# HySonLab/EquiHGNN

Measured on AMD Instinct MI355X. Metric: training molecules/sec on QM9 egnn_equihnns, higher is better.
Workload: dtype f32; 1 GPU; qm9-like synthetic molecules, --method egnn_equihnns, batch 256/rank, hidden 256, 3 layers (scripts/run_qm9_3d.sh); full training step fwd+MSE+bwd+all-reduce+Adam; batch_per_rank=256, global_batch=256, parallelism=dp1, launch=hipGraph replay (padded static shapes), collective=none (single rank)

## Files before the change

equihgnn_amd/csrc/egnn_edge.hip:

```cpp
#include <cstdlib>

#include "act.h"
#include "common.h"
#include "bf16x3.h"
#include "mfma.h"

namespace {

constexpr int KNB = 16;
constexpr int MDIM = 16;
constexpr int THREADS = 256;
constexpr int WAVES = THREADS / 64;

__device__ __forceinline__ f32x2 silu_fast2(f32x2 x) {
    const f32x2 t = x * f32x2{-1.442695041f, -1.442695041f};
    const f32x2 d = f32x2{__builtin_amdgcn_exp2f(t.x), __builtin_amdgcn_exp2f(t.y)} + f32x2{1.0f, 1.0f};
    return x * f32x2{__builtin_amdgcn_rcpf(d.x), __builtin_amdgcn_rcpf(d.y)};
}
__device__ __forceinline__ float silu_grad(float x, float* ds) {
    const float sig = sigmoid_fast(x);
    const float s = x * sig;
    *ds = fmaf(s, 1.0f - sig, sig);
    return s;
}

__device__ __forceinline__ int xcd_item(int b, int grid, int n_items, int remap) {
    if (!remap) return b < n_items ? b : -1;
    const int per = grid >> 3;
    const int item = (b & 7) * per + (b >> 3);
    return item < n_items ? item : -1;
}
static inline int xcd_grid(int n_items, int remap) { return remap ? ((n_items + 7) / 8) * 8 : n_items; }

__host__ __device__ inline int lds_row_stride(int Hp) {
    return Hp + ((24 - (Hp & 63)) + 64) % 64;
}

constexpr int FWD_THREADS = 1024;
constexpr int FWD_SPLIT = 4;
constexpr int FWD_NODES = FWD_THREADS / 64 / FWD_SPLIT;
constexpr int FWD_UB = 4;
constexpr int FWD_LD = 16 * FWD_UB + 4;
constexpr int FWD_TILE = (KNB + 1) * FWD_LD;

template <int NU>
__device__ __forceinline__ f32x4 fwd_stage(const float* __restrict__ t_rd, const float* __restrict__ t_rda,
                                           const float* __restrict__ wrow, const float* __restrict__ crow,
                                           float dd, f32x4 acc) {
    const f32x2 dd2 = {dd, dd};
#pragma unroll
    for (int u = 0; u < NU; ++u) {
        const float4 b4 = *reinterpret_cast<const float4*>(t_rd + 16 * u);
        const float4 a4 = *reinterpret_cast<const float4*>(t_rda + 16 * u);
        const float4 w4 = *reinterpret_cast<const float4*>(wrow + 16 * u);
        const float4 c4 = *reinterpret_cast<const float4*>(crow + 16 * u);
        const f32x2 h01 = f32x2{c4.x, c4.y} * dd2 + (f32x2{a4.x, a4.y} + f32x2{b4.x, b4.y});
        const f32x2 h23 = f32x2{c4.z, c4.w} * dd2 + (f32x2{a4.z, a4.w} + f32x2{b4.z, b4.w});
        const f32x2 s01 = silu_fast2(h01);
        const f32x2 s23 = silu_fast2(h23);
        acc = mfma16(s01.x, w4.x, acc);
        acc = mfma16(s01.y, w4.y, acc);
        acc = mfma16(s23.x, w4.z, acc);
        acc = mfma16(s23.y, w4.w, acc);
    }
    return acc;
}

template <bool W2_LDS>
__global__ void __launch_bounds__(FWD_THREADS)
k_edge_fwd(const float* __restrict__ ab, const float* __restrict__ wd, const float* __restrict__ w2,
           const float* __restrict__ b2, const int* __restrict__ nbr, const float* __restrict__ d2,
           float* __restrict__ m, float* __restrict__ pre2, int N, int Hp) {
    extern __shared__ __attribute__((aligned(16))) float s_mem[];
    const int ldw = W2_LDS ? lds_row_stride(Hp) : Hp;
    float* s_w2 = s_mem;
    float* s_wd = s_w2 + (W2_LDS ? MDIM * ldw : 0);
    float* s_tile = s_wd + Hp;
    if (W2_LDS) {
        for (int idx = threadIdx.x * 4; idx < MDIM * Hp; idx += FWD_THREADS * 4) {
            const int o = idx / Hp, k = idx - o * Hp;
            *reinterpret_cast<float4*>(s_w2 + o * ldw + k) = *reinterpret_cast<const float4*>(w2 + idx);
        }
    }
    for (int idx = threadIdx.x * 4; idx < Hp; idx += FWD_THREADS * 4)
        *reinterpret_cast<float4*>(s_wd + idx) = *reinterpret_cast<const float4*>(wd + idx);
    __syncthreads();
    const int lane = threadIdx.x & 63;
    const int wave = __builtin_amdgcn_readfirstlane(threadIdx.x >> 6);
    const int r = lane & 15, q = lane >> 4;
    const int slot = wave / FWD_SPLIT, part = wave % FWD_SPLIT;
    const int per = (Hp >> 4) / FWD_SPLIT;
    const int s_beg = part * per;
    const int nfull = per / FWD_UB, tail = per % FWD_UB;
    const int nstages = nfull + (tail ? 1 : 0);
    const float bo = b2[r];
    const float* __restrict__ wrow = (W2_LDS ? s_w2 : w2) + r * ldw + 4 * q + 16 * s_beg;
    const float* __restrict__ crow = s_wd + 4 * q + 16 * s_beg;
    float* tile = s_tile + wave * FWD_TILE;
    float* t_wr = tile + q * FWD_LD + 4 * r;
    const float* t_rd = tile + r * FWD_LD + 4 * q;
    const float* t_rda = tile + KNB * FWD_LD + 4 * q;
    float* t_wra = tile + KNB * FWD_LD + 4 * r;
    const int groups = (N + FWD_NODES - 1) / FWD_NODES;
    const int gpb = (groups + gridDim.x - 1) / gridDim.x;
    const int g_beg = blockIdx.x * gpb;
    const int g_end = (g_beg + gpb < groups) ? g_beg + gpb : groups;
    const int b_col0 = 16 * s_beg + 4 * r;
    if (g_beg >= g_end) return;
    const int bc0 = (b_col0 < Hp - 4) ? b_col0 : Hp - 4;
    int node_raw = g_beg * FWD_NODES + slot;
    int node = (node_raw < N) ? node_raw : N - 1;
    float dd = d2[node * KNB + r];
    const float* __restrict__ arow = ab + (int64_t)node * 2 * Hp;
    const float* __restrict__ brow0 = ab + (int64_t)nbr[node * KNB + q] * 2 * Hp + Hp;
    const float* __restrict__ brow1 = ab + (int64_t)nbr[node * KNB + 4 + q] * 2 * Hp + Hp;
    const float* __restrict__ brow2 = ab + (int64_t)nbr[node * KNB + 8 + q] * 2 * Hp + Hp;
    const float* __restrict__ brow3 = ab + (int64_t)nbr[node * KNB + 12 + q] * 2 * Hp + Hp;
    float4 nb0 = *reinterpret_cast<const float4*>(brow0 + bc0);
    float4 nb1 = *reinterpret_cast<const float4*>(brow1 + bc0);
    float4 nb2 = *reinterpret_cast<const float4*>(brow2 + bc0);
    float4 nb3 = *reinterpret_cast<const float4*>(brow3 + bc0);
    float4 na = make_float4(0.f, 0.f, 0.f, 0.f);
    if (q == 0) na = *reinterpret_cast<const float4*>(arow + bc0);
    for (int group = g_beg; group < g_end; ++group) {
        f32x4 acc = {0.f, 0.f, 0.f, 0.f};
        int j0 = 0, j1 = 0, j2 = 0, j3 = 0, node_raw_n = 0, node_n = 0;
        float dd_n = 0.f;
        for (int st = 0; st < nstages; ++st) {
            *reinterpret_cast<float4*>(t_wr) = nb0;
            *reinterpret_cast<float4*>(t_wr + 4 * FWD_LD) = nb1;
            *reinterpret_cast<float4*>(t_wr + 8 * FWD_LD) = nb2;
            *reinterpret_cast<float4*>(t_wr + 12 * FWD_LD) = nb3;
            if (q == 0) *reinterpret_cast<float4*>(t_wra) = na;
            if (st == 0) {
                const int gn = (group + 1 < g_end) ? group + 1 : group;
                node_raw_n = gn * FWD_NODES + slot;
                node_n = (node_raw_n < N) ? node_raw_n : N - 1;
                j0 = nbr[node_n * KNB + q];
                j1 = nbr[node_n * KNB + 4 + q];
                j2 = nbr[node_n * KNB + 8 + q];
                j3 = nbr[node_n * KNB + 12 + q];
                dd_n = d2[node_n * KNB + r];
            }
            const float* __restrict__ p0 = brow0;
            const float* __restrict__ p1 = brow1;
            const float* __restrict__ p2 = brow2;
            const float* __restrict__ p3 = brow3;
            const float* __restrict__ pa = arow;
            int bc;
            if (st + 1 < nstages) {
                const int off = 16 * FWD_UB * (st + 1);
                bc = (b_col0 + off < Hp - 4) ? b_col0 + off : Hp - 4;
            } else {
                asm volatile("" : "+v"(j0), "+v"(j1), "+v"(j2), "+v"(j3), "+v"(node_n));
                p0 = ab + (int64_t)j0 * 2 * Hp + Hp;
                p1 = ab + (int64_t)j1 * 2 * Hp + Hp;
                p2 = ab + (int64_t)j2 * 2 * Hp + Hp;
                p3 = ab + (int64_t)j3 * 2 * Hp + Hp;
                pa = ab + (int64_t)node_n * 2 * Hp;
                bc = bc0;
            }
            nb0 = *reinterpret_cast<const float4*>(p0 + bc);
            nb1 = *reinterpret_cast<const float4*>(p1 + bc);
            nb2 = *reinterpret_cast<const float4*>(p2 + bc);
            nb3 = *reinterpret_cast<const float4*>(p3 + bc);
            if (q == 0) na = *reinterpret_cast<const float4*>(pa + bc);
            __builtin_amdgcn_sched_barrier(0);
            const float* wr = wrow + 16 * FWD_UB * st;
            const float* cr = crow + 16 * FWD_UB * st;
            if (st < nfull) acc = fwd_stage<FWD_UB>(t_rd, t_rda, wr, cr, dd, acc);
            else if (tail == 1) acc = fwd_stage<1>(t_rd, t_rda, wr, cr, dd, acc);
            else if (tail == 2) acc = fwd_stage<2>(t_rd, t_rda, wr, cr, dd, acc);
            else acc = fwd_stage<3>(t_rd, t_rda, wr, cr, dd, acc);
            __builtin_amdgcn_sched_barrier(0);
            if (st + 1 == nstages) { brow0 = p0; brow1 = p1; brow2 = p2; brow3 = p3; arow = pa; }
        }
        if (part > 0) *reinterpret_cast<f32x4*>(tile + lane * 4) = acc;
        __syncthreads();
        if (part == 0 && node_raw < N) {
#pragma unroll
            for (int pp = 1; pp < FWD_SPLIT; ++pp)
                acc += *reinterpret_cast<const f32x4*>(tile + pp * FWD_TILE + lane * 4);
            float msum = 0.f;
#pragma unroll
            for (int g = 0; g < 4; ++g) {
                const float pv = acc[g] + bo;
                pre2[(int64_t)node * (KNB * MDIM) + (4 * q + g) * MDIM + r] = pv;
                msum += silu_fast(pv);
            }
            msum += __shfl_xor(msum, 16, 64);
            msum += __shfl_xor(msum, 32, 64);
            if (q == 0) m[(int64_t)node * MDIM + r] = msum;
        }
        __syncthreads();
        node_raw = node_raw_n;
        node = node_n;
        dd = dd_n;
    }
}

constexpr int edge_planes(int np) { return np == 6 ? 3 : (np == 3 ? 2 : 1); }

constexpr int F2_SPLIT = 4;
constexpr int F2_LD = 32 + 4;
constexpr int F2_TILE = (KNB + 1) * F2_LD;
constexpr int F2_MAXSTEPS = 9;

template <int PL>
__device__ __forceinline__ void split8(const float (&v)[8], uint4& p0, uint4& p1, uint4& p2) {
    split_pair_n<PL>(v[0], v[1], p0.x, p1.x, p2.x);
    split_pair_n<PL>(v[2], v[3], p0.y, p1.y, p2.y);
    split_pair_n<PL>(v[4], v[5], p0.z, p1.z, p2.z);
    split_pair_n<PL>(v[6], v[7], p0.w, p1.w, p2.w);
}

template <int NS, int THREADS_, bool W2_LDS, int NP>
__global__ void __launch_bounds__(THREADS_)
k_edge_fwd_x3(const float* __restrict__ ab, const float* __restrict__ wd, const float* __restrict__ w2,
              const float* __restrict__ b2, const int* __restrict__ nbr, const float* __restrict__ d2,
              float* __restrict__ m, float* __restrict__ pre2, int N, int Hp, int n_items, int remap) {
    extern __shared__ __attribute__((aligned(16))) float s_mem[];
    constexpr int NWAVES = THREADS_ / 64, NODES = NWAVES / F2_SPLIT, PL = edge_planes(NP);
    const int item = xcd_item((int)blockIdx.x, (int)gridDim.x, n_items, remap);
    if (item < 0) return;
    const int total = Hp >> 5;
    float* s_wd = s_mem;
    float* s_tile = s_wd + Hp;
    uint4* s_w2 = reinterpret_cast<uint4*>(s_tile + NWAVES * F2_TILE);
    for (int idx = threadIdx.x * 4; idx < Hp; idx += THREADS_ * 4)
        *reinterpret_cast<float4*>(s_wd + idx) = *reinterpret_cast<const float4*>(wd + idx);
    const int lane = threadIdx.x & 63;
    const int wave = __builtin_amdgcn_readfirstlane(threadIdx.x >> 6);
    const int r = lane & 15, q = lane >> 4;
    const int slot = wave / F2_SPLIT, part = wave % F2_SPLIT;
    const int per = (total + F2_SPLIT - 1) / F2_SPLIT;
    const int s_beg = part * per;
    const int cnt = (total - s_beg < per) ? (total - s_beg > 0 ? total - s_beg : 0) : per;
    auto w2_frag = [&](int step, uint4& p0, uint4& p1, uint4& p2) {
        float v[8];
        const int k0 = 32 * step + 8 * q;
        const float4 x0 = *reinterpret_cast<const float4*>(w2 + r * Hp + k0);
        const float4 x1 = *reinterpret_cast<const float4*>(w2 + r * Hp + k0 + 4);
        v[0] = x0.x; v[1] = x0.y; v[2] = x0.z; v[3] = x0.w; v[4] = x1.x; v[5] = x1.y; v[6] = x1.z; v[7] = x1.w;
        split8<PL>(v, p0, p1, p2);
    };
    uint4 wf[W2_LDS ? 1 : NS][3];
    if constexpr (W2_LDS) {
        for (int step = wave; step < total; step += NWAVES) {
            uint4 p0, p1, p2;
            w2_frag(step, p0, p1, p2);
            s_w2[(step * 3 + 0) * 64 + lane] = p0;
            if constexpr (PL > 1) s_w2[(step * 3 + 1) * 64 + lane] = p1;
            if constexpr (PL > 2) s_w2[(step * 3 + 2) * 64 + lane] = p2;
        }
    } else {
#pragma unroll
        for (int s = 0; s < NS; ++s) {
            if (s < cnt) w2_frag(s_beg + s, wf[s][0], wf[s][1], wf[s][2]);
            else wf[s][0] = wf[s][1] = wf[s][2] = make_uint4(0u, 0u, 0u, 0u);
        }
    }
    __syncthreads();
    const float bo = b2[r];
    float* tile = s_tile + wave * F2_TILE;
    const int lrow = lane >> 3, piece = lane & 7;
    float* t_wr0 = tile + lrow * F2_LD + 4 * piece;
    float* t_wr1 = t_wr0 + 8 * F2_LD;
    float* t_wra = tile + KNB * F2_LD + 4 * piece;
    const float* t_rd = tile + r * F2_LD + 8 * q;
    const float* t_rda = tile + KNB * F2_LD + 8 * q;
    const int groups = (N + NODES - 1) / NODES;
    const int gpb = (groups + n_items - 1) / n_items;
    const int g_beg = item * gpb;
    const int g_end = (g_beg + gpb < groups) ? g_beg + gpb : groups;
    if (g_beg >= g_end) return;
    const int col0 = 32 * s_beg + 4 * piece;
    int node_raw = g_beg * NODES + slot;
    int node = (node_raw < N) ? node_raw : N - 1;
    float dd = d2[node * KNB + r];
    const float* __restrict__ arow = ab + (int64_t)node * 2 * Hp;
    const float* __restrict__ brow0 = ab + (int64_t)nbr[node * KNB + lrow] * 2 * Hp + Hp;
    const float* __restrict__ brow1 = ab + (int64_t)nbr[node * KNB + 8 + lrow] * 2 * Hp + Hp;
    float4 nb0 = f4_zero(), nb1 = f4_zero(), na = f4_zero();
    if (cnt > 0) {
        nb0 = *reinterpret_cast<const float4*>(brow0 + col0);
        nb1 = *reinterpret_cast<const float4*>(brow1 + col0);
        if (lane < 8) na = *reinterpret_cast<const float4*>(arow + col0);
    }
    for (int group = g_beg; group < g_end; ++group) {
        f32x4 acc = {0.f, 0.f, 0.f, 0.f};
        int j0 = 0, j1 = 0, node_raw_n = 0, node_n = 0;
        float dd_n = 0.f;
        {
            const int gn = (group + 1 < g_end) ? group + 1 : group;
            node_raw_n = gn * NODES + slot;
            node_n = (node_raw_n < N) ? node_raw_n : N - 1;
            j0 = nbr[node_n * KNB + lrow];
            j1 = nbr[node_n * KNB + 8 + lrow];
            dd_n = d2[node_n * KNB + r];
        }
#pragma unroll
        for (int st = 0; st < NS; ++st) {
            if (st < cnt) {
                *reinterpret_cast<float4*>(t_wr0) = nb0;
                *reinterpret_cast<float4*>(t_wr1) = nb1;
                if (lane < 8) *reinterpret_cast<float4*>(t_wra) = na;
                const float* __restrict__ p0 = brow0;
                const float* __restrict__ p1 = brow1;
                const float* __restrict__ pa = arow;
                int bc;
                if (st + 1 < cnt) {
                    bc = col0 + 32 * (st + 1);
                } else {
                    asm volatile("" : "+v"(j0), "+v"(j1), "+v"(node_n));
                    p0 = ab + (int64_t)j0 * 2 * Hp + Hp;
                    p1 = ab + (int64_t)j1 * 2 * Hp + Hp;
                    pa = ab + (int64_t)node_n * 2 * Hp;
                    bc = col0;
                }
                nb0 = *reinterpret_cast<const float4*>(p0 + bc);
                nb1 = *reinterpret_cast<const float4*>(p1 + bc);
                if (lane < 8) na = *reinterpret_cast<const float4*>(pa + bc);
                if (st + 1 >= cnt) { brow0 = p0; brow1 = p1; arow = pa; }
                __builtin_amdgcn_sched_barrier(0);
                const float* cr = s_wd + 32 * (s_beg + st) + 8 * q;
                const float4 b0 = *reinterpret_cast<const float4*>(t_rd), b1 = *reinterpret_cast<const float4*>(t_rd + 4);
                const float4 a0 = *reinterpret_cast<const float4*>(t_rda), a1 = *reinterpret_cast<const float4*>(t_rda + 4);
                const float4 c0 = *reinterpret_cast<const float4*>(cr), c1 = *reinterpret_cast<const float4*>(cr + 4);
#ifdef EDGE_ABLATE
                acc[0] += (b0.x + b1.w) + (a0.y + a1.z) + (c0.x + c1.x);
                __builtin_amdgcn_sched_barrier(0);
                continue;
#endif
                const f32x2 dd2 = {dd, dd};
                const f32x2 s01 = silu_fast2(f32x2{c0.x, c0.y} * dd2 + (f32x2{a0.x, a0.y} + f32x2{b0.x, b0.y}));
                const f32x2 s23 = silu_fast2(f32x2{c0.z, c0.w} * dd2 + (f32x2{a0.z, a0.w} + f32x2{b0.z, b0.w}));
                const f32x2 s45 = silu_fast2(f32x2{c1.x, c1.y} * dd2 + (f32x2{a1.x, a1.y} + f32x2{b1.x, b1.y}));
                const f32x2 s67 = silu_fast2(f32x2{c1.z, c1.w} * dd2 + (f32x2{a1.z, a1.w} + f32x2{b1.z, b1.w}));
                uint4 p0_, p1_, p2_;
                split_pair_n<PL>(s01.x, s01.y, p0_.x, p1_.x, p2_.x);
                split_pair_n<PL>(s23.x, s23.y, p0_.y, p1_.y, p2_.y);
                split_pair_n<PL>(s45.x, s45.y, p0_.z, p1_.z, p2_.z);
                split_pair_n<PL>(s67.x, s67.y, p0_.w, p1_.w, p2_.w);
                const bf16x8 x0 = __builtin_bit_cast(bf16x8, p0_), x1 = __builtin_bit_cast(bf16x8, p1_), x2 = __builtin_bit_cast(bf16x8, p2_);
                uint4 q0, q1 = make_uint4(0u, 0u, 0u, 0u), q2 = q1;
                if constexpr (W2_LDS) {
                    const uint4* wp = s_w2 + (s_beg + st) * 3 * 64 + lane;
                    q0 = wp[0];
                    if constexpr (PL > 1) q1 = wp[64];
                    if constexpr (PL > 2) q2 = wp[128];
                } else {
                    q0 = wf[st][0]; q1 = wf[st][1]; q2 = wf[st][2];
                }
                const bf16x8 w0 = __builtin_bit_cast(bf16x8, q0), w1 = __builtin_bit_cast(bf16x8, q1), w2p = __builtin_bit_cast(bf16x8, q2);
                if constexpr (NP == 6) {
                    acc = __builtin_amdgcn_mfma_f32_16x16x32_bf16(x1, w1, acc, 0, 0, 0);
                    acc = __builtin_amdgcn_mfma_f32_16x16x32_bf16(x0, w2p, acc, 0, 0, 0);
                    acc = __builtin_amdgcn_mfma_f32_16x16x32_bf16(x2, w0, acc, 0, 0, 0);
                    acc = __builtin_amdgcn_mfma_f32_16x16x32_bf16(x0, w1, acc, 0, 0, 0);
                    acc = __builtin_amdgcn_mfma_f32_16x16x32_bf16(x1, w0, acc, 0, 0, 0);
                } else if constexpr (NP == 3) {
                    acc = __builtin_amdgcn_mfma_f32_16x16x32_bf16(x1, w0, acc, 0, 0, 0);
                    acc = __builtin_amdgcn_mfma_f32_16x16x32_bf16(x0, w1, acc, 0, 0, 0);
                }
                acc = __builtin_amdgcn_mfma_f32_16x16x32_bf16(x0, w0, acc, 0, 0, 0);
                __builtin_amdgcn_sched_barrier(0);
            }
        }
        if (part > 0) *reinterpret_cast<f32x4*>(tile + lane * 4) = acc;
        __syncthreads();
        if (part == 0 && node_raw < N) {
#pragma unroll
            for (int pp = 1; pp < F2_SPLIT; ++pp)
                acc += *reinterpret_cast<const f32x4*>(tile + pp * F2_TILE + lane * 4);
            float msum = 0.f;
#pragma unroll
            for (int g = 0; g < 4; ++g) {
                const float pv = acc[g] + bo;
                pre2[(int64_t)node * (KNB * MDIM) + (4 * q + g) * MDIM + r] = pv;
                msum += silu_fast(pv);
            }
            msum += __shfl_xor(msum, 16, 64);
            msum += __shfl_xor(msum, 32, 64);
            if (q == 0) m[(int64_t)node * MDIM + r] = msum;
        }
        __syncthreads();
        node_raw = node_raw_n;
        node = node_n;
        dd = dd_n;
    }
}

template <int NP>
__device__ __forceinline__ f32x4 mfma16_planes(const Planes4& a, const Planes4& b, f32x4 c) {
    if constexpr (NP == 3) {
        c = mfma16_bf16(a.p1, b.p0, c);
        c = mfma16_bf16(a.p0, b.p1, c);
    }
    return mfma16_bf16(a.p0, b.p0, c);
}
template <int NP>
__device__ __forceinline__ void w2_planes(const float4& w0, const float4& w1, const float4& w2v, const float4& w3, Planes4& c0,
                                          Planes4& c1, Planes4& c2, Planes4& c3) {
    constexpr int PL = edge_planes(NP);
    c0 = split_quad<PL>(w0.x, w1.x, w2v.x, w3.x);
    c1 = split_quad<PL>(w0.y, w1.y, w2v.y, w3.y);
    c2 = split_quad<PL>(w0.z, w1.z, w2v.z, w3.z);
    c3 = split_quad<PL>(w0.w, w1.w, w2v.w, w3.w);
}
constexpr int BW_RESIDENT = 768;

__host__ __device__ inline int bw_chunks(int64_t n_items, int tiles) {
    int64_t c = BW_RESIDENT / tiles;
    if (c < 1) c = 1;
    const int64_t most = (n_items + WAVES - 1) / WAVES;
    if (c > most) c = most;
    return (int)(c < 1 ? 1 : c);
}

__global__ void __launch_bounds__(THREADS)
k_edge_bwd_prep(const float* __restrict__ pre2, const float* __restrict__ dm, float* __restrict__ dpre2,
                float* __restrict__ dpre2_t, const int* __restrict__ t_perm, const int* __restrict__ nbr,
                const float* __restrict__ d2, int4* __restrict__ rec, float* __restrict__ slab_b2, int N, int64_t dm_ld) {
    const int64_t E = (int64_t)N * KNB;
    for (int64_t p = (int64_t)blockIdx.x * THREADS + threadIdx.x; p < E; p += (int64_t)gridDim.x * THREADS) {
        const int e = t_perm[p];
        rec[p] = make_int4(e, nbr[e], __float_as_int(d2[e]), 0);
    }
    const int lane = threadIdx.x & 63, wave = threadIdx.x >> 6;
    float4 acc_b2 = f4_zero();
    for (int node = blockIdx.x * WAVES + wave; node < N; node += gridDim.x * WAVES) {
        const int jj = lane >> 2, o0 = (lane & 3) * 4;
        const float4 p4 = *reinterpret_cast<const float4*>(pre2 + (int64_t)node * 256 + lane * 4);
        const float4 g4 = *reinterpret_cast<const float4*>(dm + (int64_t)node * dm_ld + o0);
        float ds;
        float4 d4;
        silu_grad(p4.x, &ds); d4.x = g4.x * ds;
        silu_grad(p4.y, &ds); d4.y = g4.y * ds;
        silu_grad(p4.z, &ds); d4.z = g4.z * ds;
        silu_grad(p4.w, &ds); d4.w = g4.w * ds;
        *reinterpret_cast<float4*>(dpre2 + (int64_t)node * 256 + lane * 4) = d4;
        float* __restrict__ t = dpre2_t + (int64_t)node * 256 + jj;
        t[(o0 + 0) * KNB] = d4.x;
        t[(o0 + 1) * KNB] = d4.y;
        t[(o0 + 2) * KNB] = d4.z;
        t[(o0 + 3) * KNB] = d4.w;
        f4_add(acc_b2, d4);
    }
    if (slab_b2) {
#pragma unroll
        for (int off = 4; off < 64; off <<= 1) {
            acc_b2.x += __shfl_xor(acc_b2.x, off); acc_b2.y += __shfl_xor(acc_b2.y, off);
            acc_b2.z += __shfl_xor(acc_b2.z, off); acc_b2.w += __shfl_xor(acc_b2.w, off);
        }
        __shared__ float4 s_b2[WAVES][4];
        if (lane < 4) s_b2[wave][lane] = acc_b2;
        __syncthreads();
        if (threadIdx.x < 4) {
            float4 v = s_b2[0][threadIdx.x];
            for (int w = 1; w < WAVES; ++w) f4_add(v, s_b2[w][threadIdx.x]);
            *reinterpret_cast<float4*>(slab_b2 + (int64_t)blockIdx.x * MDIM + 4 * threadIdx.x) = v;
        }
    }
}

struct RecvOps {
    float4 pa;
    float4 pt;
    float4 a;
    float4 dd;
    float4 b0, b1, b2, b3;
};

__device__ __forceinline__ void recv_load(RecvOps& o, const float* __restrict__ ab, const float* __restrict__ d2,
                                          const float* __restrict__ dpre2, const float* __restrict__ dpre2_t,
                                          int node, int4 nb, int Hp, int k4, int r, int q) {
    o.pa = *reinterpret_cast<const float4*>(dpre2 + (int64_t)node * 256 + r * MDIM + 4 * q);
    o.pt = *reinterpret_cast<const float4*>(dpre2_t + (int64_t)node * 256 + r * KNB + 4 * q);
    o.a = *reinterpret_cast<const float4*>(ab + (int64_t)node * 2 * Hp + k4);
    o.dd = *reinterpret_cast<const float4*>(d2 + (int64_t)node * KNB + 4 * q);
    o.b0 = *reinterpret_cast<const float4*>(ab + (int64_t)nb.x * 2 * Hp + Hp + k4);
    o.b1 = *reinterpret_cast<const float4*>(ab + (int64_t)nb.y * 2 * Hp + Hp + k4);
    o.b2 = *reinterpret_cast<const float4*>(ab + (int64_t)nb.z * 2 * Hp + Hp + k4);
    o.b3 = *reinterpret_cast<const float4*>(ab + (int64_t)nb.w * 2 * Hp + Hp + k4);
}

template <int NP>
__device__ __forceinline__ float recv_column(float a, float wdc, const float4& dd, float b0, float b1, float b2,
                                             float b3, const f32x4& gk, const float4& pt, const Planes4& ptp, float& acc_wd,
                                             f32x4& acc_w) {
    float ds0, ds1, ds2, ds3;
    const float s0 = silu_grad(fmaf(wdc, dd.x, a + b0), &ds0);
    const float s1 = silu_grad(fmaf(wdc, dd.y, a + b1), &ds1);
    const float s2 = silu_grad(fmaf(wdc, dd.z, a + b2), &ds2);
    const float s3 = silu_grad(fmaf(wdc, dd.w, a + b3), &ds3);
    const float dh0 = gk[0] * ds0, dh1 = gk[1] * ds1, dh2 = gk[2] * ds2, dh3 = gk[3] * ds3;
    acc_wd = fmaf(dh0, dd.x, acc_wd);
    acc_wd = fmaf(dh1, dd.y, acc_wd);
    acc_wd = fmaf(dh2, dd.z, acc_wd);
    acc_wd = fmaf(dh3, dd.w, acc_wd);
    if constexpr (NP == 6) {
        acc_w = mfma16(pt.x, s0, acc_w);
        acc_w = mfma16(pt.y, s1, acc_w);
        acc_w = mfma16(pt.z, s2, acc_w);
        acc_w = mfma16(pt.w, s3, acc_w);
    } else {
        acc_w = mfma16_planes<NP>(ptp, split_quad<edge_planes(NP)>(s0, s1, s2, s3), acc_w);
    }
    return (dh0 + dh1) + (dh2 + dh3);
}

template <int NP>
__global__ void __launch_bounds__(THREADS)
k_edge_bwd_recv(const float* __restrict__ ab, const float* __restrict__ wd, const float* __restrict__ w2,
                const int* __restrict__ nbr, const float* __restrict__ d2, const float* __restrict__ dpre2,
                const float* __restrict__ dpre2_t, float* __restrict__ dab, float* __restrict__ slab_w2,
                float* __restrict__ slab_wd, int N, int Hp, int tiles, int chunk_nodes, int n_items, int remap) {
    __shared__ __attribute__((aligned(16))) float s_red[WAVES - 1][64 * 20];
    const int lane = threadIdx.x & 63;
    const int wave = __builtin_amdgcn_readfirstlane(threadIdx.x >> 6);
    const int r = lane & 15, q = lane >> 4;
    const int item = xcd_item((int)blockIdx.x, (int)gridDim.x, n_items, remap);
    if (item < 0) return;
    const int T = item % tiles, chunk = item / tiles;
    const int base = chunk * chunk_nodes;
    const int cnt = (N - base < chunk_nodes) ? (N - base) : chunk_nodes;
    const int k4 = 64 * T + 4 * r;
    const float4 w0 = *reinterpret_cast<const float4*>(w2 + (4 * q + 0) * Hp + k4);
    const float4 w1 = *reinterpret_cast<const float4*>(w2 + (4 * q + 1) * Hp + k4);
    const float4 w2v = *reinterpret_cast<const float4*>(w2 + (4 * q + 2) * Hp + k4);
    const float4 w3 = *reinterpret_cast<const float4*>(w2 + (4 * q + 3) * Hp + k4);
    const float4 wd4 = *reinterpret_cast<const float4*>(wd + k4);
    Planes4 wp0 = {}, wp1 = {}, wp2 = {}, wp3 = {};
    if constexpr (NP != 6) w2_planes<NP>(w0, w1, w2v, w3, wp0, wp1, wp2, wp3);
    f32x4 aw0 = {0.f, 0.f, 0.f, 0.f}, aw1 = aw0, aw2 = aw0, aw3 = aw0;
    float ad0 = 0.f, ad1 = 0.f, ad2 = 0.f, ad3 = 0.f;
    const int last = cnt - 1;
    int n = wave;
    if (n < cnt) {
        const int4* __restrict__ nbr4 = reinterpret_cast<const int4*>(nbr);
        auto clampn = [&](int x) { return base + (x < last ? x : last); };
        int4 nb_next = nbr4[(int64_t)clampn(n) * 4 + q];
        RecvOps nx;
        recv_load(nx, ab, d2, dpre2, dpre2_t, clampn(n), nb_next, Hp, k4, r, q);
        nb_next = nbr4[(int64_t)clampn(n + WAVES) * 4 + q];
        for (; n < cnt; n += WAVES) {
            const RecvOps cur = nx;
            const int node = base + n;
            recv_load(nx, ab, d2, dpre2, dpre2_t, clampn(n + WAVES), nb_next, Hp, k4, r, q);
            nb_next = nbr4[(int64_t)clampn(n + 2 * WAVES) * 4 + q];
            __builtin_amdgcn_sched_barrier(0);
#ifdef EDGE_ABLATE
            {
                const float t = (cur.pa.x + cur.pt.y) + (cur.a.x + cur.dd.y) + ((cur.b0.x + cur.b1.y) + (cur.b2.z + cur.b3.w));
                if (q == 0) *reinterpret_cast<float4*>(dab + (int64_t)node * 2 * Hp + k4) = make_float4(t, t, t, t);
                ad0 += t;
                continue;
            }
#endif
            f32x4 g0 = {0.f, 0.f, 0.f, 0.f}, g1 = g0, g2 = g0, g3 = g0;
            Planes4 ptp = {};
            if constexpr (NP == 6) {
                g0 = mfma16(cur.pa.x, w0.x, g0); g1 = mfma16(cur.pa.x, w0.y, g1);
                g2 = mfma16(cur.pa.x, w0.z, g2); g3 = mfma16(cur.pa.x, w0.w, g3);
                g0 = mfma16(cur.pa.y, w1.x, g0); g1 = mfma16(cur.pa.y, w1.y, g1);
                g2 = mfma16(cur.pa.y, w1.z, g2); g3 = mfma16(cur.pa.y, w1.w, g3);
                g0 = mfma16(cur.pa.z, w2v.x, g0); g1 = mfma16(cur.pa.z, w2v.y, g1);
                g2 = mfma16(cur.pa.z, w2v.z, g2); g3 = mfma16(cur.pa.z, w2v.w, g3);
                g0 = mfma16(cur.pa.w, w3.x, g0); g1 = mfma16(cur.pa.w, w3.y, g1);
                g2 = mfma16(cur.pa.w, w3.z, g2); g3 = mfma16(cur.pa.w, w3.w, g3);
            } else {
                const Planes4 pap = split_quad<edge_planes(NP)>(cur.pa.x, cur.pa.y, cur.pa.z, cur.pa.w);
                g0 = mfma16_planes<NP>(pap, wp0, g0); g1 = mfma16_planes<NP>(pap, wp1, g1);
                g2 = mfma16_planes<NP>(pap, wp2, g2); g3 = mfma16_planes<NP>(pap, wp3, g3);
                ptp = split_quad<edge_planes(NP)>(cur.pt.x, cur.pt.y, cur.pt.z, cur.pt.w);
            }
            float da0 = recv_column<NP>(cur.a.x, wd4.x, cur.dd, cur.b0.x, cur.b1.x, cur.b2.x, cur.b3.x, g0, cur.pt, ptp, ad0, aw0);
            float da1 = recv_column<NP>(cur.a.y, wd4.y, cur.dd, cur.b0.y, cur.b1.y, cur.b2.y, cur.b3.y, g1, cur.pt, ptp, ad1, aw1);
            float da2 = recv_column<NP>(cur.a.z, wd4.z, cur.dd, cur.b0.z, cur.b1.z, cur.b2.z, cur.b3.z, g2, cur.pt, ptp, ad2, aw2);
            float da3 = recv_column<NP>(cur.a.w, wd4.w, cur.dd, cur.b0.w, cur.b1.w, cur.b2.w, cur.b3.w, g3, cur.pt, ptp, ad3, aw3);
            da0 += __shfl_xor(da0, 16, 64); da1 += __shfl_xor(da1, 16, 64);
            da2 += __shfl_xor(da2, 16, 64); da3 += __shfl_xor(da3, 16, 64);
            da0 += __shfl_xor(da0, 32, 64); da1 += __shfl_xor(da1, 32, 64);
            da2 += __shfl_xor(da2, 32, 64); da3 += __shfl_xor(da3, 32, 64);
            if (q == 0)
                *reinterpret_cast<float4*>(dab + (int64_t)node * 2 * Hp + k4) = make_float4(da0, da1, da2, da3);
            __builtin_amdgcn_sched_barrier(0);
        }
    }
    ad0 += __shfl_xor(ad0, 16, 64); ad1 += __shfl_xor(ad1, 16, 64);
    ad2 += __shfl_xor(ad2, 16, 64); ad3 += __shfl_xor(ad3, 16, 64);
    ad0 += __shfl_xor(ad0, 32, 64); ad1 += __shfl_xor(ad1, 32, 64);
    ad2 += __shfl_xor(ad2, 32, 64); ad3 += __shfl_xor(ad3, 32, 64);
    if (wave > 0) {
        float* p = &s_red[wave - 1][lane * 20];
        *reinterpret_cast<f32x4*>(p) = aw0;
        *reinterpret_cast<f32x4*>(p + 4) = aw1;
        *reinterpret_cast<f32x4*>(p + 8) = aw2;
        *reinterpret_cast<f32x4*>(p + 12) = aw3;
        *reinterpret_cast<float4*>(p + 16) = make_float4(ad0, ad1, ad2, ad3);
    }
    __syncthreads();
    if (wave == 0) {
#pragma unroll
        for (int w = 0; w < WAVES - 1; ++w) {
            const float* p = &s_red[w][lane * 20];
            aw0 += *reinterpret_cast<const f32x4*>(p);
            aw1 += *reinterpret_cast<const f32x4*>(p + 4);
            aw2 += *reinterpret_cast<const f32x4*>(p + 8);
            aw3 += *reinterpret_cast<const f32x4*>(p + 12);
            const float4 d = *reinterpret_cast<const float4*>(p + 16);
            ad0 += d.x; ad1 += d.y; ad2 += d.z; ad3 += d.w;
        }
        float* __restrict__ sw = slab_w2 + (int64_t)chunk * (MDIM + 1) * Hp;
#pragma unroll
        for (int g = 0; g < 4; ++g)
            *reinterpret_cast<float4*>(sw + (4 * q + g) * Hp + k4) = make_float4(aw0[g], aw1[g], aw2[g], aw3[g]);
        if (q == 0)
            *reinterpret_cast<float4*>(slab_wd + (int64_t)chunk * (MDIM + 1) * Hp + k4) = make_float4(ad0, ad1, ad2, ad3);
    }
}

constexpr int SEND_LD = 68;

struct SendOps {
    float4 pa;
    float4 a0, a1, a2, a3;
    float4 b0, b1, b2, b3;
    float dd0, dd1, dd2, dd3;
};

__device__ __forceinline__ void send_load(SendOps& o, const float* __restrict__ ab,
                                          const float* __restrict__ dpre2, int4 rc, int Hp, int k4, int q) {
    o.pa = *reinterpret_cast<const float4*>(dpre2 + (int64_t)rc.x * MDIM + 4 * q);
    const int e0 = __shfl(rc.x, 4 * q + 0, 64), e1 = __shfl(rc.x, 4 * q + 1, 64);
    const int e2 = __shfl(rc.x, 4 * q + 2, 64), e3 = __shfl(rc.x, 4 * q + 3, 64);
    const int j0 = __shfl(rc.y, 4 * q + 0, 64), j1 = __shfl(rc.y, 4 * q + 1, 64);
    const int j2 = __shfl(rc.y, 4 * q + 2, 64), j3 = __shfl(rc.y, 4 * q + 3, 64);
    o.dd0 = __int_as_float(__shfl(rc.z, 4 * q + 0, 64));
    o.dd1 = __int_as_float(__shfl(rc.z, 4 * q + 1, 64));
    o.dd2 = __int_as_float(__shfl(rc.z, 4 * q + 2, 64));
    o.dd3 = __int_as_float(__shfl(rc.z, 4 * q + 3, 64));
    o.a0 = *reinterpret_cast<const float4*>(ab + (int64_t)(e0 >> 4) * 2 * Hp + k4);
    o.a1 = *reinterpret_cast<const float4*>(ab + (int64_t)(e1 >> 4) * 2 * Hp + k4);
    o.a2 = *reinterpret_cast<const float4*>(ab + (int64_t)(e2 >> 4) * 2 * Hp + k4);
    o.a3 = *reinterpret_cast<const float4*>(ab + (int64_t)(e3 >> 4) * 2 * Hp + k4);
    o.b0 = *reinterpret_cast<const float4*>(ab + (int64_t)j0 * 2 * Hp + Hp + k4);
    o.b1 = *reinterpret_cast<const float4*>(ab + (int64_t)j1 * 2 * Hp + Hp + k4);
    o.b2 = *reinterpret_cast<const float4*>(ab + (int64_t)j2 * 2 * Hp + Hp + k4);
    o.b3 = *reinterpret_cast<const float4*>(ab + (int64_t)j3 * 2 * Hp + Hp + k4);
}

__device__ __forceinline__ float4 send_row(const float4& wd4, float dd, const float4& a4, const float4& b4,
                                           float gk0, float gk1, float gk2, float gk3) {
    float ds;
    float4 dh;
    silu_grad(fmaf(wd4.x, dd, a4.x + b4.x), &ds); dh.x = gk0 * ds;
    silu_grad(fmaf(wd4.y, dd, a4.y + b4.y), &ds); dh.y = gk1 * ds;
    silu_grad(fmaf(wd4.z, dd, a4.z + b4.z), &ds); dh.z = gk2 * ds;
    silu_grad(fmaf(wd4.w, dd, a4.w + b4.w), &ds); dh.w = gk3 * ds;
    return dh;
}

template <int NP>
__global__ void __launch_bounds__(THREADS)
k_edge_bwd_send(const float* __restrict__ ab, const float* __restrict__ wd, const float* __restrict__ w2,
                const float* __restrict__ dpre2, const int* __restrict__ t_rowptr, const int4* __restrict__ rec,
                float* __restrict__ dab, int N, int Hp, int tiles, int chunk_senders, int n_items, int remap) {
    __shared__ __attribute__((aligned(16))) float s_tile[WAVES][KNB * SEND_LD];
    const int lane = threadIdx.x & 63;
    const int wave = __builtin_amdgcn_readfirstlane(threadIdx.x >> 6);
    const int r = lane & 15, q = lane >> 4;
    const int item = xcd_item((int)blockIdx.x, (int)gridDim.x, n_items, remap);
    if (item < 0) return;
    const int T = item % tiles, chunk = item / tiles;
    const int k4 = 64 * T + 4 * r;
    const int c_beg = chunk * chunk_senders;
    const int c_cnt = (N - c_beg < chunk_senders) ? (N - c_beg) : chunk_senders;
    const int per = (c_cnt + WAVES - 1) / WAVES;
    const int s_beg = c_beg + ((wave * per < c_cnt) ? wave * per : c_cnt);
    const int s_end = c_beg + (((wave + 1) * per < c_cnt) ? (wave + 1) * per : c_cnt);
    if (s_beg >= s_end) return;
    const int p_beg = t_rowptr[s_beg], p_end = t_rowptr[s_end];
    float* drow = dab + Hp + 64 * T + lane;
    if (p_beg == p_end) {
        for (int sj = s_beg; sj < s_end; ++sj) drow[(int64_t)sj * 2 * Hp] = 0.f;
        return;
    }
    const float4 w0 = *reinterpret_cast<const float4*>(w2 + (4 * q + 0) * Hp + k4);
    const float4 w1 = *reinterpret_cast<const float4*>(w2 + (4 * q + 1) * Hp + k4);
    const float4 w2v = *reinterpret_cast<const float4*>(w2 + (4 * q + 2) * Hp + k4);
    const float4 w3 = *reinterpret_cast<const float4*>(w2 + (4 * q + 3) * Hp + k4);
    const float4 wd4 = *reinterpret_cast<const float4*>(wd + k4);
    Planes4 wp0 = {}, wp1 = {}, wp2 = {}, wp3 = {};
    if constexpr (NP != 6) w2_planes<NP>(w0, w1, w2v, w3, wp0, wp1, wp2, wp3);
    float* tile = s_tile[wave];
    int rp_base = s_beg;
    int rp = t_rowptr[((rp_base + lane < N) ? rp_base + lane : N - 1) + 1];
    int cur = s_beg;
    int cur_end = __builtin_amdgcn_readlane(rp, 0);
    float run = 0.f;
    const int p_last = p_end - 1;
    auto pos = [&](int p) { return (p + r < p_last) ? p + r : p_last; };
    int4 rc_next = rec[pos(p_beg)];
    SendOps nx;
    send_load(nx, ab, dpre2, rc_next, Hp, k4, q);
    rc_next = rec[pos(p_beg + KNB)];
    for (int p0 = p_beg; p0 < p_end; p0 += KNB) {
        const SendOps cur_ops = nx;
        send_load(nx, ab, dpre2, rc_next, Hp, k4, q);
        rc_next = rec[pos(p0 + 2 * KNB)];
        __builtin_amdgcn_sched_barrier(0);
        const bool live_r = p0 + r < p_end;
        const float4 pa = live_r ? cur_ops.pa : make_float4(0.f, 0.f, 0.f, 0.f);
#ifdef EDGE_ABLATE
        {
            run += (pa.x + cur_ops.dd0) + ((cur_ops.a0.x + cur_ops.a1.y) + (cur_ops.a2.z + cur_ops.a3.w)) +
                   ((cur_ops.b0.x + cur_ops.b1.y) + (cur_ops.b2.z + cur_ops.b3.w));
            if ((p0 & 255) == 0) drow[(int64_t)cur * 2 * Hp] = run;
            continue;
        }
#endif
        f32x4 g0 = {0.f, 0.f, 0.f, 0.f}, g1 = g0, g2 = g0, g3 = g0;
        if constexpr (NP == 6) {
            g0 = mfma16(pa.x, w0.x, g0); g1 = mfma16(pa.x, w0.y, g1); g2 = mfma16(pa.x, w0.z, g2); g3 = mfma16(pa.x, w0.w, g3);
            g0 = mfma16(pa.y, w1.x, g0); g1 = mfma16(pa.y, w1.y, g1); g2 = mfma16(pa.y, w1.z, g2); g3 = mfma16(pa.y, w1.w, g3);
            g0 = mfma16(pa.z, w2v.x, g0); g1 = mfma16(pa.z, w2v.y, g1); g2 = mfma16(pa.z, w2v.z, g2); g3 = mfma16(pa.z, w2v.w, g3);
            g0 = mfma16(pa.w, w3.x, g0); g1 = mfma16(pa.w, w3.y, g1); g2 = mfma16(pa.w, w3.z, g2); g3 = mfma16(pa.w, w3.w, g3);
        } else {
            const Planes4 pap = split_quad<edge_planes(NP)>(pa.x, pa.y, pa.z, pa.w);
            g0 = mfma16_planes<NP>(pap, wp0, g0); g1 = mfma16_planes<NP>(pap, wp1, g1);
            g2 = mfma16_planes<NP>(pap, wp2, g2); g3 = mfma16_planes<NP>(pap, wp3, g3);
        }
        float* trow = tile + 4 * q * SEND_LD + 4 * r;
        *reinterpret_cast<float4*>(trow) = send_row(wd4, cur_ops.dd0, cur_ops.a0, cur_ops.b0, g0[0], g1[0], g2[0], g3[0]);
        *reinterpret_cast<float4*>(trow + SEND_LD) = send_row(wd4, cur_ops.dd1, cur_ops.a1, cur_ops.b1, g0[1], g1[1], g2[1], g3[1]);
        *reinterpret_cast<float4*>(trow + 2 * SEND_LD) = send_row(wd4, cur_ops.dd2, cur_ops.a2, cur_ops.b2, g0[2], g1[2], g2[2], g3[2]);
        *reinterpret_cast<float4*>(trow + 3 * SEND_LD) = send_row(wd4, cur_ops.dd3, cur_ops.a3, cur_ops.b3, g0[3], g1[3], g2[3], g3[3]);
        float v[KNB];
#pragma unroll
        for (int row = 0; row < KNB; ++row) v[row] = tile[row * SEND_LD + lane];
        const int rows = (p_end - p0 < KNB) ? (p_end - p0) : KNB;
#pragma unroll
        for (int row = 0; row < KNB; ++row) {
            if (row < rows) {
                while (p0 + row >= cur_end) {
                    drow[(int64_t)cur * 2 * Hp] = run;
                    run = 0.f;
                    ++cur;
                    if (cur - rp_base >= 64) {
                        rp_base += 64;
                        rp = t_rowptr[((rp_base + lane < N) ? rp_base + lane : N - 1) + 1];
                    }
                    cur_end = __builtin_amdgcn_readlane(rp, cur - rp_base);
                }
                run += v[row];
            }
        }
        __builtin_amdgcn_sched_barrier(0);
    }
    for (; cur < s_end; ++cur) {
        drow[(int64_t)cur * 2 * Hp] = run;
        run = 0.f;
    }
}

inline int edge_xcd_remap() {
    static const int v = [] { const char* e = std::getenv("EQH_EDGE_XCD"); return (e && e[0] == '0') ? 0 : 1; }();
    return v;
}

int check_common(int64_t N, int Hp) {
    if (N < 0 || Hp <= 0) return EQH_ERR_ARG;
    if (Hp & 63) return EQH_ERR_ALIGN;
    if (N * 2 * (int64_t)Hp >= ((int64_t)1 << 31) * 4) return EQH_ERR_RANGE;
    if (N * KNB >= ((int64_t)1 << 31)) return EQH_ERR_RANGE;
    return EQH_OK;
}

template <int NP>
int fwd_x3_launch(const float* ab, const float* wd, const float* w2, const float* b2, const int32_t* nbr, const float* d2,
                  int64_t N, int32_t Hp, float* m, float* pre2, hipStream_t stream, int per, bool w8, size_t lds2) {
    const int threads = w8 ? 512 : 1024;
    const int items2 = eqh_grid_for(N, threads / 64 / F2_SPLIT, 256);
    const int remap = edge_xcd_remap();
    const int grid2 = xcd_grid(items2, remap);
    static bool attr2 = false;
#define F2_ATTR(NS_)                                                                                                          \
    (hipFuncSetAttribute(reinterpret_cast<const void*>(k_edge_fwd_x3<NS_, 1024, true, NP>), hipFuncAttributeMaxDynamicSharedMemorySize, \
                         160 * 1024) == hipSuccess)
    if (!attr2) {
        if (!(F2_ATTR(1) && F2_ATTR(2) && F2_ATTR(3) && F2_ATTR(5) && F2_ATTR(9))) return EQH_ERR_LAUNCH;
        attr2 = true;
    }
#undef F2_ATTR
#define F2_LAUNCH(NS_)                                                                                                         \
    do {                                                                                                                   \
        if (w8) hipLaunchKernelGGL((k_edge_fwd_x3<NS_, 512, false, NP>), dim3(grid2), dim3(512), lds2, stream, ab, wd, w2, b2, nbr, d2, m, \
                                   pre2, (int)N, (int)Hp, items2, remap);                                                  \
        else hipLaunchKernelGGL((k_edge_fwd_x3<NS_, 1024, true, NP>), dim3(grid2), dim3(1024), lds2, stream, ab, wd, w2, b2, nbr, d2, m, \
                                pre2, (int)N, (int)Hp, items2, remap);                                                     \
    } while (0)
    if (per <= 1) F2_LAUNCH(1);
    else if (per <= 2) F2_LAUNCH(2);
    else if (per <= 3) F2_LAUNCH(3);
    else if (per <= 5) F2_LAUNCH(5);
    else F2_LAUNCH(9);
#undef F2_LAUNCH
    EQH_CHECK_LAUNCH();
    return EQH_OK;
}

}

extern "C" int egnn_edge_fwd_p(const float* ab, const float* wd, const float* w2, const float* b2,
                               const int32_t* nbr, const float* d2, int64_t N, int32_t Hp, float* m,
                               float* pre2, void* stream_, int32_t products) {
    if (products != 6 && products != 3 && products != 1) return EQH_ERR_ARG;
    int rc = check_common(N, Hp);
    if (rc) return rc;
    if (N == 0) return EQH_OK;
    if (!ab || !wd || !w2 || !b2 || !nbr || !d2 || !m || !pre2) return EQH_ERR_ARG;
    if (!eqh_aligned16(ab) || !eqh_aligned16(wd) || !eqh_aligned16(w2)) return EQH_ERR_ALIGN;
    hipStream_t stream = static_cast<hipStream_t>(stream_);
    static const bool use_f32 = [] { const char* e = std::getenv("EQH_EDGE_F32"); return e && e[0] == '1'; }();
    const int per = ((Hp >> 5) + F2_SPLIT - 1) / F2_SPLIT;
    if (!use_f32 && per <= F2_MAXSTEPS && (size_t)N * 2 * (size_t)Hp < ((size_t)1 << 31)) {
        static const bool w8 = [] { const char* e = std::getenv("EQH_EDGE_W8"); return e && e[0] == '1'; }();
        const int threads = w8 ? 512 : 1024;
        const size_t lds2 = ((size_t)Hp + (size_t)(threads / 64) * F2_TILE) * sizeof(float) + (w8 ? 0 : (size_t)(Hp >> 5) * 3 * 64 * 16);
        if (lds2 > 160 * 1024) return EQH_ERR_RANGE;
        if (products == 6) return fwd_x3_launch<6>(ab, wd, w2, b2, nbr, d2, N, Hp, m, pre2, stream, per, w8, lds2);
        if (products == 3) return fwd_x3_launch<3>(ab, wd, w2, b2, nbr, d2, N, Hp, m, pre2, stream, per, w8, lds2);
        return fwd_x3_launch<1>(ab, wd, w2, b2, nbr, d2, N, Hp, m, pre2, stream, per, w8, lds2);
    }
    const size_t lds_rest = ((size_t)Hp + (size_t)(FWD_THREADS / 64) * FWD_TILE) * sizeof(float);
    const size_t lds_w2 = (size_t)MDIM * lds_row_stride(Hp) * sizeof(float);
    const bool w2_lds = lds_rest + lds_w2 <= 160 * 1024;
    const size_t lds = lds_rest + (w2_lds ? lds_w2 : 0);
    if (lds > 160 * 1024) return EQH_ERR_RANGE;
    static bool attr_set = false;
    if (!attr_set) {
        if (hipFuncSetAttribute(reinterpret_cast<const void*>(k_edge_fwd<true>),
                                hipFuncAttributeMaxDynamicSharedMemorySize, 160 * 1024) != hipSuccess ||
            hipFuncSetAttribute(reinterpret_cast<const void*>(k_edge_fwd<false>),
                                hipFuncAttributeMaxDynamicSharedMemorySize, 160 * 1024) != hipSuccess)
            return EQH_ERR_LAUNCH;
        attr_set = true;
    }
    const int grid = eqh_grid_for(N, FWD_NODES, 256);
    if (w2_lds)
        hipLaunchKernelGGL(k_edge_fwd<true>, dim3(grid), dim3(FWD_THREADS), lds, stream, ab, wd, w2, b2, nbr, d2,
                           m, pre2, (int)N, (int)Hp);
    else
        hipLaunchKernelGGL(k_edge_fwd<false>, dim3(grid), dim3(FWD_THREADS), lds, stream, ab, wd, w2, b2, nbr, d2,
                           m, pre2, (int)N, (int)Hp);
    EQH_CHECK_LAUNCH();
    return EQH_OK;
}

extern "C" int egnn_edge_fwd(const float* ab, const float* wd, const float* w2, const float* b2,
                             const int32_t* nbr, const float* d2, int64_t N, int32_t Hp, float* m,
                             float* pre2, void* stream_) {
    return egnn_edge_fwd_p(ab, wd, w2, b2, nbr, d2, N, Hp, m, pre2, stream_, 6);
}

static inline int prep_blocks(int64_t N) { return eqh_grid_for(N, WAVES, 2048); }

extern "C" size_t egnn_edge_bwd_workspace_bytes(int64_t N, int32_t Hp) {
    if (N < 0 || Hp <= 0) return 0;
    const int chunks = bw_chunks(N, Hp >> 6);
    return ((size_t)chunks * (size_t)(MDIM + 1) * (size_t)Hp + (size_t)(N > 0 ? N : 1) * 256 +
            (size_t)(N > 0 ? N : 1) * KNB * 4 + (size_t)prep_blocks(N) * MDIM) * sizeof(float);
}

extern "C" int egnn_edge_bwd_p(const float* ab, const float* wd, const float* w2, const int32_t* nbr,
                               const float* d2, const float* pre2, const float* dm, int64_t dm_ld,
                               const int32_t* t_rowptr, const int32_t* t_perm, int64_t N, int32_t Hp,
                               float* dab, float* dwd, float* dw2, float* dpre2, float* db2,
                               int32_t db2_accumulate, int32_t dw_accumulate, void* workspace, size_t workspace_bytes,
                               void* stream_, int32_t products) {
    if (products != 6 && products != 3 && products != 1) return EQH_ERR_ARG;
    int rc = check_common(N, Hp);
    if (rc) return rc;
    if (!dwd || !dw2) return EQH_ERR_ARG;
    hipStream_t stream = static_cast<hipStream_t>(stream_);
    if (N == 0) {
        if (!dw_accumulate && (eqh_zero_async(dwd, Hp, stream) || eqh_zero_async(dw2, (int64_t)MDIM * Hp, stream)))
            return EQH_ERR_LAUNCH;
        if (db2 && !db2_accumulate && eqh_zero_async(db2, MDIM, stream)) return EQH_ERR_LAUNCH;
        return EQH_OK;
    }
    if (!ab || !wd || !w2 || !nbr || !d2 || !pre2 || !dm || !t_rowptr || !t_perm || !dab || !dpre2 ||
        !workspace)
        return EQH_ERR_ARG;
    if (!eqh_aligned16(ab) || !eqh_aligned16(wd) || !eqh_aligned16(w2) || !eqh_aligned16(nbr) ||
        !eqh_aligned16(d2) || !eqh_aligned16(pre2) || !eqh_aligned16(dm) || !eqh_aligned16(dpre2) ||
        !eqh_aligned16(dab) || !eqh_aligned16(workspace))
        return EQH_ERR_ALIGN;
    if (workspace_bytes < egnn_edge_bwd_workspace_bytes(N, Hp)) return EQH_ERR_ARG;
    if (dm_ld < MDIM || (dm_ld & 3)) return EQH_ERR_ARG;
    const int tiles = Hp >> 6;
    const int chunks = bw_chunks(N, tiles);
    const int chunk_items = (int)((N + chunks - 1) / chunks);
    const int used = (int)((N + chunk_items - 1) / chunk_items);
    float* slab_w2 = static_cast<float*>(workspace);
    float* slab_wd = slab_w2 + (size_t)MDIM * Hp;
    float* dpre2_t = slab_w2 + (size_t)chunks * (MDIM + 1) * Hp;
    int4* rec = reinterpret_cast<int4*>(dpre2_t + (size_t)N * 256);
    float* slab_b2 = db2 ? reinterpret_cast<float*>(rec + (size_t)N * KNB) : nullptr;
    const int pblocks = prep_blocks(N);
    hipLaunchKernelGGL(k_edge_bwd_prep, dim3(pblocks), dim3(THREADS), 0, stream, pre2, dm,
                       dpre2, dpre2_t, t_perm, nbr, d2, rec, slab_b2, (int)N, dm_ld);
    EQH_CHECK_LAUNCH();
    if (db2) {
        rc = eqh_reduce_slabs_async(slab_b2, pblocks, MDIM, db2, stream, db2_accumulate);
        if (rc) return rc;
    }
    const int remap = edge_xcd_remap();
    const auto recv = products == 6 ? k_edge_bwd_recv<6> : (products == 3 ? k_edge_bwd_recv<3> : k_edge_bwd_recv<1>);
    const auto send = products == 6 ? k_edge_bwd_send<6> : (products == 3 ? k_edge_bwd_send<3> : k_edge_bwd_send<1>);
    hipLaunchKernelGGL(recv, dim3(xcd_grid(used * tiles, remap)), dim3(THREADS), 0, stream, ab, wd, w2, nbr, d2, dpre2,
                       dpre2_t, dab, slab_w2, slab_wd, (int)N, (int)Hp, tiles, chunk_items, used * tiles, remap);
    EQH_CHECK_LAUNCH();
    hipLaunchKernelGGL(send, dim3(xcd_grid(used * tiles, remap)), dim3(THREADS), 0, stream, ab, wd, w2, dpre2, t_rowptr,
                       rec, dab, (int)N, (int)Hp, tiles, chunk_items, used * tiles, remap);
    EQH_CHECK_LAUNCH();
    return eqh_reduce_slabs3_async(slab_w2, used, (int64_t)(MDIM + 1) * Hp, dw2, dwd, dwd, (int64_t)MDIM * Hp, Hp,
                                   dw_accumulate ? 1 : 0, stream);
}

extern "C" int egnn_edge_bwd(const float* ab, const float* wd, const float* w2, const int32_t* nbr,
                             const float* d2, const float* pre2, const float* dm, int64_t dm_ld,
                             const int32_t* t_rowptr, const int32_t* t_perm, int64_t N, int32_t Hp,
                             float* dab, float* dwd, float* dw2, float* dpre2, float* db2,
                             int32_t db2_accumulate, int32_t dw_accumulate, void* workspace, size_t workspace_bytes,
                             void* stream_) {
    return egnn_edge_bwd_p(ab, wd, w2, nbr, d2, pre2, dm, dm_ld, t_rowptr, t_perm, N, Hp, dab, dwd, dw2, dpre2, db2,
                           db2_accumulate, dw_accumulate, workspace, workspace_bytes, stream_, 6);
}
```

equihgnn_amd/layers.py:

```python
from __future__ import annotations

import torch
import torch.nn as nn
import torch.nn.functional as F

from . import ops
from .batch import ATOM_FEATURE_DIMS
from .index import HyperIndex


def _make_norm(kind: str, width: int) -> nn.Module:
    if kind == "ln":
        return nn.LayerNorm(width)
    if kind == "bn":
        return nn.BatchNorm1d(width)
    if kind == "None":
        return nn.Identity()
    raise AssertionError(f"Normalization must be bn/ln/None, got {kind}")


class AtomEncoder(nn.Module):

    def __init__(self, emb_dim: int):
        super().__init__()
        self.atom_embedding_list = nn.ModuleList()
        offs, run = [], 0
        for d in ATOM_FEATURE_DIMS:
            emb = nn.Embedding(d, emb_dim)
            nn.init.xavier_uniform_(emb.weight.data)
            self.atom_embedding_list.append(emb)
            offs.append(run)
            run += d
        self.offsets = tuple(offs)

    def forward(self, x):
        return ops.embed_sum(x, [e.weight for e in self.atom_embedding_list], self.offsets)


class BondEncoder(nn.Embedding):

    def forward(self, idx):
        return ops.embed_sum(idx.reshape(-1, 1), self.weight, (0,))


class MLP(nn.Module):

    def __init__(self, in_channels, hidden_channels, out_channels, num_layers,
                 dropout=0.5, Normalization="bn", InputNorm=False):
        super().__init__()
        self.lins = nn.ModuleList()
        self.normalizations = nn.ModuleList()
        self.InputNorm = InputNorm
        self.normalizations.append(_make_norm(Normalization, in_channels) if InputNorm else nn.Identity())
        widths = [in_channels] + [hidden_channels] * (num_layers - 1) + [out_channels]
        for i in range(num_layers):
            self.lins.append(nn.Linear(widths[i], widths[i + 1]))
            if i < num_layers - 1:
                self.normalizations.append(_make_norm(Normalization, widths[i + 1]))
        self.dropout = dropout

    def reset_parameters(self):
        for lin in self.lins:
            lin.reset_parameters()
        for n in self.normalizations:
            if not isinstance(n, nn.Identity):
                n.reset_parameters()

    @staticmethod
    def _norm(norm, h, mask):
        if isinstance(norm, nn.BatchNorm1d) and h.dim() == 2:
            return batch_norm_rows(norm, h, mask)
        return norm(h)

    @property
    def has_batch_norm(self) -> bool:
        return any(isinstance(n, nn.BatchNorm1d) for n in self.normalizations)

    def hidden(self, h, start: int, mask=None):
        last = len(self.lins) - 1
        for i in range(start, last):
            if i > start:
                h = ops.linear(h, self.lins[i].weight, self.lins[i].bias) if h.is_cuda else self.lins[i](h)
            h = F.relu(h)
            h = self._norm(self.normalizations[i + 1], h, mask)
            h = F.dropout(h, p=self.dropout, training=self.training)
        return h

    def takes_first(self, x) -> bool:
        return len(self.lins) > 1 and not self.InputNorm and self._fusable(x)

    @property
    def drop_p(self) -> float:
        return float(self.dropout) if (self.training and self.dropout > 0) else 0.0

    def _fusable(self, x):
        return (x.is_cuda and x.dim() == 2 and (self.drop_p == 0.0 or ops.FUSED_DROPOUT)
                and all(isinstance(n, nn.LayerNorm) for n in self.normalizations[1:])
                and all(l.out_features % 4 == 0 and l.out_features <= 1024 for l in self.lins[:-1]))

    def forward(self, x, first=None, mask=None):
        x = self._norm(self.normalizations[0], x, mask)
        if len(self.lins) == 1:
            return ops.linear(x, self.lins[0].weight, self.lins[0].bias)
        if self._fusable(x):
            for i in range(len(self.lins) - 1):
                lin, norm = self.lins[i], self.normalizations[i + 1]
                h = first if (i == 0 and first is not None) else ops.linear(x, lin.weight)
                x = ops.bias_relu_ln(h, lin.bias, norm.weight, norm.bias, norm.eps, p=self.drop_p)
            return ops.linear(x, self.lins[-1].weight, self.lins[-1].bias)
        h = self.hidden(ops.linear(x, self.lins[0].weight, self.lins[0].bias), 0, mask)
        return ops.linear(h, self.lins[-1].weight, self.lins[-1].bias)


def _row_weight(out_csr, has_row, aggr, dtype):
    if aggr == "mean":
        return has_row
    return (out_csr.rowptr[1:] - out_csr.rowptr[:-1]).to(dtype)[:, None]


def _pair_message(mlp: MLP, a, b, idx_a32, idx_b32, csr_a, csr_b, out_csr, out_key32, has_row, aggr,
                  residual=None, pa=None, inc_mask=None):
    if mlp.InputNorm or mlp.has_batch_norm:
        h = torch.cat((ops.gather_rows(a, idx_a32, csr_a), ops.gather_rows(b, idx_b32, csr_b)), -1)
        out = ops.reduce_entries(mlp(h, mask=inc_mask), out_csr, out_key32, aggr)
        return out if residual is None else residual[0] * out + residual[2]
    lin0 = mlp.lins[0]
    ca = a.shape[-1]
    cin = lin0.weight.shape[1]
    if pa is None:
        pa = ops.linear(a, lin0.weight, None, (0, ca))
    qb = ops.linear(b, lin0.weight, lin0.bias, (ca, cin))
    norm = mlp.normalizations[1] if len(mlp.lins) > 1 else None
    fused = (len(mlp.lins) == 2 and isinstance(norm, nn.LayerNorm) and pa.dim() == 2
             and pa.shape[-1] % 4 == 0 and pa.shape[-1] <= 1024
             and (mlp.drop_p == 0.0 or (ops.FUSED_DROPOUT and pa.is_cuda)))
    last = mlp.lins[-1]
    if fused:
        s = ops.incidence_ln_reduce(pa, qb, norm.weight, norm.bias, idx_a32, idx_b32, csr_a, csr_b,
                                    out_csr, out_key32, aggr, norm.eps, p=mlp.drop_p)
        if residual is not None:
            return ops.linear_add(s, last.weight, residual[1], residual[0])
        return torch.addcmul(ops.linear(s, last.weight), _row_weight(out_csr, has_row, aggr, s.dtype), last.bias)
    h = ops.gather_rows(pa, idx_a32, csr_a) + ops.gather_rows(qb, idx_b32, csr_b)
    if len(mlp.lins) == 1:
        out = ops.reduce_entries(h, out_csr, out_key32, aggr)
        return out if residual is None else residual[0] * out + residual[2]
    h = mlp.hidden(h, 0)
    s = ops.reduce_entries(h, out_csr, out_key32, aggr)
    if residual is not None:
        return ops.linear_add(s, last.weight, residual[1], residual[0])
    return ops.linear(s, last.weight) + last.bias * _row_weight(out_csr, has_row, aggr, s.dtype)


class MHNNConv(nn.Module):

    def __init__(self, hid_dim, mlp1_layers=1, mlp2_layers=1, mlp3_layers=1, mlp4_layers=1,
                 aggr="mean", dropout=0.0, normalization="None", input_norm=False):
        super().__init__()
        mk = lambda n: (MLP(hid_dim * 2, hid_dim, hid_dim, n, dropout=dropout, Normalization=normalization, InputNorm=input_norm)
                        if n > 0 else None)
        self.W1, self.W2, self.W3, self.W4 = mk(mlp1_layers), mk(mlp2_layers), mk(mlp3_layers), mk(mlp4_layers)
        self.aggr = aggr
        self.dropout = dropout

    def reset_parameters(self):
        for w in (self.W1, self.W2, self.W3, self.W4):
            if w is not None:
                w.reset_parameters()

    def forward(self, X, E, index: HyperIndex):
        ix = index
        if ops.mhnn_panel_supported(X, E, self):
            return ops.mhnn_conv_panel(self, X, E, ix)
        mk = ix.pad_masks()
        if self.W1 is None:
            m_e = ops.reduce_entries(ops.gather_rows(E, ix.e32, ix.by_e), ix.by_e, ix.e32, self.aggr)
        else:
            m_e = _pair_message(self.W1, X, E, ix.v32, ix.e32, ix.by_v, ix.by_e, ix.by_e, ix.e32,
                                ix.has_e, self.aggr, inc_mask=mk[2])
        E = m_e if self.W2 is None else self.W2(torch.cat((E, m_e), -1), mask=mk[1])
        if self.W3 is None:
            m_v = ops.reduce_gathered(E, ix.by_v, ix.by_e, self.aggr)
        else:
            m_v = _pair_message(self.W3, X, E, ix.v32, ix.e32, ix.by_v, ix.by_e, ix.by_v, ix.v32,
                                ix.has_v, self.aggr, inc_mask=mk[2])
        X = m_v if self.W4 is None else self.W4(torch.cat((X, m_v), -1), mask=mk[0])
        return X, E


def real_row_mask(data, like):
    nb = getattr(data, "num_real_graphs", None)
    if nb is None or nb >= data.y.shape[0]:
        return None
    return (data.batch < nb).to(like.dtype).unsqueeze(-1)


def batch_norm_rows(bn: nn.BatchNorm1d, x, mask, relu: bool = False):
    if ops.batch_norm_rows_supported(x, bn):
        return ops.batch_norm_rows(x, mask, bn, relu=relu)
    if relu:
        return torch.relu(batch_norm_rows(bn, x, mask))
    if mask is None or not bn.training or not bn.track_running_stats or bn.momentum is None:
        return bn(x)
    n = mask.sum()
    mean = (x * mask).sum(0) / n
    xc = x - mean
    var = (xc * xc * mask).sum(0) / n
    y = xc * torch.rsqrt(var + bn.eps) * bn.weight + bn.bias
    with torch.no_grad():
        bn.running_mean.lerp_(mean, bn.momentum)
        bn.running_var.lerp_(var * (n / (n - 1.0)), bn.momentum)
        bn.num_batches_tracked.add_(1)
    return y


MERGE_LINEARS = True


class MHNNSConv(nn.Module):

    def __init__(self, hid_dim, mlp1_layers=1, mlp2_layers=1, mlp3_layers=1, aggr="mean",
                 alpha=0.5, dropout=0.0, normalization="None", input_norm=False):
        super().__init__()
        mk = lambda cin, n: (MLP(cin, hid_dim, hid_dim, n, dropout=dropout, Normalization=normalization, InputNorm=input_norm)
                             if n > 0 else None)
        self.W1, self.W2 = mk(hid_dim, mlp1_layers), mk(hid_dim * 2, mlp2_layers)
        if mlp3_layers > 0:
            self.W3 = mk(hid_dim, mlp3_layers)
        else:
            self.W = nn.Identity()
        self.aggr = aggr
        self.alpha = alpha
        self.dropout = dropout

    def _mlps(self):
        return [w for w in (self.W1, self.W2, getattr(self, "W3", None)) if w is not None]

    @property
    def plain(self) -> bool:
        ws = (self.W1, self.W2, getattr(self, "W3", None))
        return any(w is None for w in ws) or any(w.InputNorm or w.has_batch_norm for w in ws)

    def reset_parameters(self):
        for w in self._mlps():
            w.reset_parameters()

    def residual(self, X0, index: HyperIndex, passthrough: bool = False):
        a = self.alpha
        if X0.is_cuda and X0.dim() == 2 and X0.shape[-1] % 4 == 0 and X0.dtype == torch.float32:
            mode = 1 if self.aggr == "mean" else 2
            if passthrough:
                c, x0p = ops.residual_mix(X0, self.W2.lins[-1].bias, index.by_v.rowptr, mode, a, passthrough=True)
                return (1.0 - a, c, None, x0p)
            return (1.0 - a, ops.residual_mix(X0, self.W2.lins[-1].bias, index.by_v.rowptr, mode, a), None)
        x0a = X0 * a
        if X0.dim() != 2:
            return (1.0 - a, None, x0a)
        rows = _row_weight(index.by_v, index.has_v, self.aggr, X0.dtype)
        return (1.0 - a, torch.addcmul(x0a, rows, self.W2.lins[-1].bias, value=1.0 - a), x0a)

    def prepare(self, X0, index: HyperIndex):
        if self.plain:
            return None
        if X0.is_cuda and X0.dim() == 2 and len(self.W2.lins) > 1:
            if self._mergeable(X0):
                return self._prepare_merged(self.residual(X0, index, passthrough=True), X0)
            return self.residual(X0, index)
        return None

    def _mergeable(self, X) -> bool:
        two = all(len(w.lins) == 2 for w in (self.W1, self.W2, self.W3))
        return (MERGE_LINEARS and two and self.aggr == "mean" and X.is_cuda and X.dim() == 2 and X.dtype == torch.float32
                and self.W1._fusable(X) and self.W2._fusable(X) and self.W3._fusable(X)
                and not (self.W1.InputNorm or self.W2.InputNorm or self.W3.InputNorm))

    def _prepare_merged(self, res, X0):
        c_dim = self.W1.lins[0].weight.shape[1]
        (w12, b12), (w23, _) = ops.merged_weights([
            (self.W2.lins[0].weight, self.W1.lins[1].weight, self.W1.lins[1].bias, self.W2.lins[0].bias, (c_dim, 2 * c_dim)),
            (self.W3.lins[0].weight, self.W2.lins[1].weight, None, None, None)])
        cw = ops.linear(res[1], self.W3.lins[0].weight)
        cw, fan = ops.fanout(cw)
        return {"scale": res[0], "w12": w12, "b12": b12, "w23": w23, "cw": cw, "fan": fan, "x0": X0, "x0_pass": res[3]}

    def _forward_merged(self, X, ix: HyperIndex, m, relu_out=False):
        c = X.shape[-1]
        if X is m["x0"]:
            X = m["x0_pass"]
        W1, W2, W3 = self.W1, self.W2, self.W3
        h1, pa = ops.linear2(X, W1.lins[0].weight, None, W2.lins[0].weight, (0, c))
        n1, n2, n3 = W1.normalizations[1], W2.normalizations[1], W3.normalizations[1]
        hbar = ops.gather_ln_reduce(h1, W1.lins[0].bias, n1.weight, n1.bias, ix.by_e, ix.by_v, "mean", n1.eps, p=W1.drop_p)
        qb = ops.linear(hbar, m["w12"], m["b12"])
        s = ops.incidence_ln_reduce(pa, qb, n2.weight, n2.bias, ix.v32, ix.e32, ix.by_v, ix.by_e, ix.by_v, ix.v32,
                                    "mean", n2.eps, p=W2.drop_p)
        x = ops.linear_add_relu_ln(s, m["w23"], m["cw"], m["scale"], W3.lins[0].bias, n3.weight, n3.bias, n3.eps, fan=m["fan"],
                                   p=W3.drop_p)
        return ops.linear(x, W3.lins[1].weight, W3.lins[1].bias, relu=relu_out)

    def stack_supported(self, X, residual, p_x: float = 0.0) -> bool:
        if not isinstance(residual, dict) or self.plain:
            return False
        probs = (p_x,) + tuple(w.drop_p for w in (self.W1, self.W2, self.W3))
        if (self.training and self.dropout > 0) or any(p > 0 for p in probs):
            if not ops.stack_dropout_supported(probs + ((self.dropout,) if self.training else ())):
                return False
        return ops.conv_stack_supported(X, self.W1.lins[0].weight.shape[0])

    def forward_stack(self, X, index: HyperIndex, residual, n_layers: int, relu_out: bool, p_x: float = 0.0):
        m = residual
        if X is m["x0"]:
            X = m["x0_pass"]
        return ops.merged_conv_stack(X, m["cw"], self.W1, self.W2, self.W3, m["w12"], m["b12"], m["w23"], index, n_layers,
                                     m["scale"], relu_out, p_x=p_x)

    def forward(self, X, index: HyperIndex, X0, residual=None, relu_out=False):
        ix = index
        if isinstance(residual, dict):
            return self._forward_merged(X, ix, residual, relu_out)
        assert not relu_out
        if self.plain:
            mk = ix.pad_masks()
            w1x = X if self.W1 is None else self.W1(X, mask=mk[0])
            x_e = ops.reduce_gathered(w1x, ix.by_e, ix.by_v, self.aggr)
            if self.W2 is None:
                x_v = ops.reduce_gathered(x_e, ix.by_v, ix.by_e, self.aggr)
            else:
                x_v = _pair_message(self.W2, X, x_e, ix.v32, ix.e32, ix.by_v, ix.by_e, ix.by_v, ix.v32, ix.has_v, self.aggr,
                                    inc_mask=mk[2])
            return self.W3(torch.lerp(x_v, X0, self.alpha), mask=mk[0])
        fused = X.is_cuda and X.dim() == 2 and len(self.W2.lins) > 1
        pa = None
        if fused and self.W1.takes_first(X) and not self.W2.InputNorm:
            c = X.shape[-1]
            h1, pa = ops.linear2(X, self.W1.lins[0].weight, None, self.W2.lins[0].weight, (0, c))
            w1x = self.W1(X, first=h1)
        else:
            w1x = self.W1(X)
        x_e = ops.reduce_gathered(w1x, ix.by_e, ix.by_v, self.aggr)
        if fused:
            res = residual if residual is not None else self.residual(X0, ix)
            mixed = _pair_message(self.W2, X, x_e, ix.v32, ix.e32, ix.by_v, ix.by_e, ix.by_v, ix.v32,
                                  ix.has_v, self.aggr, residual=res, pa=pa)
            return self.W3(mixed)
        x_v = _pair_message(self.W2, X, x_e, ix.v32, ix.e32, ix.by_v, ix.by_e, ix.by_v, ix.v32,
                            ix.has_v, self.aggr)
        return self.W3(torch.lerp(x_v, X0, self.alpha))


class CoorsNorm(nn.Module):

    def __init__(self, scale_init=1.0):
        super().__init__()
        self.scale = nn.Parameter(torch.full((1,), float(scale_init)))


class EGNN(nn.Module):

    def __init__(self, dim, m_dim=16, num_nearest_neighbors=16, init_eps=1e-3,
                 norm_coors_scale_init=1e-2):
        super().__init__()
        e_in = 2 * dim + 1
        self.dim, self.m_dim, self.k = dim, m_dim, num_nearest_neighbors
        self.edge_mlp = nn.Sequential(nn.Linear(e_in, 2 * e_in), nn.Identity(), nn.SiLU(),
                                      nn.Linear(2 * e_in, m_dim), nn.SiLU())
        self.node_norm = nn.LayerNorm(dim)
        self.coors_norm = CoorsNorm(norm_coors_scale_init)
        self.node_mlp = nn.Sequential(nn.Linear(dim + m_dim, 2 * dim), nn.Identity(), nn.SiLU(),
                                      nn.Linear(2 * dim, dim))
        self.coors_mlp = nn.Sequential(nn.Linear(m_dim, 4 * m_dim), nn.Identity(), nn.SiLU(),
                                       nn.Linear(4 * m_dim, 1))
        for mod in self.modules():
            if type(mod) is nn.Linear:
                nn.init.normal_(mod.weight, std=init_eps)

    def forward(self, feats, coors, index: HyperIndex):
        c = self.dim
        nbr, d2, csr_t = index.knn(coors, self.k, 0)
        lin1, lin2 = self.edge_mlp[0], self.edge_mlp[3]
        hdim = lin1.weight.shape[0]
        hp = hdim + (-hdim) % 64
        w_cat, b_cat, w_d, w2 = ops.egnn_pack_weights(lin1.weight, lin1.bias, lin2.weight, hp)
        nn_ = self.node_norm
        n0, n3 = self.node_mlp[0], self.node_mlp[3]
        fold = (ops.NODE_LN_FOLD and ops.USE_NODE_PANEL and feats.dim() == 2 and feats.is_cuda and feats.dtype == torch.float32
                and tuple(nn_.normalized_shape) == (c,) and nn_.elementwise_affine and nn_.bias is not None
                and ops.panel_supported(c) and tuple(n0.weight.shape) == (2 * c, c + 16) and tuple(n3.weight.shape) == (c, 2 * c)
                and feats.shape[0] > 0 and self.edge_mlp[3].weight.shape[0] == 16)
        if fold:
            ab, normed, res = ops.egnn_feats(feats, w_cat, b_cat, None)
        elif feats.dim() == 2 and c % 4 == 0 and c <= 1024:
            ab, normed, res = ops.egnn_feats(feats, w_cat, b_cat, nn_)
        else:
            ab, normed, res = ops.linear(feats, w_cat, b_cat), nn_(feats), feats
        m_i = ops.egnn_edge(ab, w_d, w2, lin2.bias, nbr, d2, csr_t)
        ops.signal_point()
        if fold:
            return ops.egnn_node_mlp_ln(normed, m_i, n0, n3, nn_)
        if ops.USE_NODE_PANEL and ops.egnn_node_mlp_supported(normed, m_i, n0, n3):
            return ops.egnn_node_mlp(normed, m_i, res, n0, n3)
        node_in = torch.cat((normed, m_i), -1)
        hid = F.silu(ops.linear(node_in, n0.weight, n0.bias))
        return ops.linear(hid, n3.weight, n3.bias) + res


def pool_sum(x, index: HyperIndex):
    return ops.reduce_entries(x, index.pool, index.batch32, "sum")


def head_spec(head):
    return head[3] if len(head) > 3 else None


def head_loss(out, head):
    if head is None:
        return out
    nb = head[1] or out.shape[0]
    return ops.regression_loss(out[:nb], head[0][:nb], head_spec(head))


def readout(mlp_out, x, index: HyperIndex, taps=None, head=None, p_x=0.0, drop=None):
    if head is not None and taps is None:
        ops.signal_point("readout")
        x2 = x.reshape(-1, x.shape[-1])
        plain = p_x == 0.0 and ops.readout_mse_supported(x2, mlp_out)
        if head[0].is_cuda and (plain or ops.readout_mse_drop_supported(x2, mlp_out, p_x)):
            loss, _ = ops.readout_mse(x2, index.pool.rowptr, mlp_out, head[0], head[1],
                                      unit_grad=bool(head[2]) if len(head) > 2 else False, p_x=p_x, loss=head_spec(head))
            ops.signal_point("after_readout")
            return loss
    if drop is not None:
        x = drop(x)
    xp = pool_sum(x, index)
    if taps is not None:
        taps["pool"] = xp
    return head_loss(mlp_out(xp, mask=index.pad_masks()[3]).view(-1), head)
```

equihgnn_amd/ops/egnn.py:

```python
from __future__ import annotations

import os

import torch

from .. import hip, precision
from ._base import (
    ACC_PARAMS, LINEAR_PARAMS, _DEFER, _acc_target, _f32c, _hand_out, _note_acc, _ptr, _require_gpu, _rows_ld, _stream,
    _workspace, timed)
from .aggregate import (CSR)
from .products import (USE_X6, X6_WGRAD_ROWS, gemm, gemm_supported, mm_nn, mm_nt)
from .grads import (_merged_acc, _wgrad_deferred, colsum)
from .panel import backward_as_forward


class _EgnnEdge(torch.autograd.Function):

    @staticmethod
    def forward(ctx, ab, wd, w2, b2, nbr, d2, csr_t: CSR, b2_param=None, w_refs=None):
        _require_gpu(ab, "egnn_edge")
        ab, wd, w2, b2 = _f32c(ab), _f32c(wd), _f32c(w2), _f32c(b2)
        N, Hp = ab.shape[0], ab.shape[1] // 2
        if nbr.shape != (N, 16) or w2.shape != (16, Hp) or wd.shape != (Hp,) or b2.shape != (16,):
            raise ValueError("egnn_edge: shapes must be ab[N,2Hp] wd[Hp] w2[16,Hp] b2[16] nbr[N,16]")
        m = torch.empty((N, 16), dtype=torch.float32, device=ab.device)
        pre2 = torch.empty((N, 16, 16), dtype=torch.float32, device=ab.device)
        ctx.products = products = precision.edge_products()
        timed("egnn_edge_fwd", N * 16 * Hp * 32,
              lambda: hip.check(hip.lib().egnn_edge_fwd_p(_ptr(ab), _ptr(wd), _ptr(w2), _ptr(b2), _ptr(nbr), _ptr(d2), N, Hp,
                                                          _ptr(m), _ptr(pre2), _stream(ab.device), products), "egnn_edge_fwd"))
        ctx.save_for_backward(ab, wd, w2, pre2)
        ctx.nbr, ctx.d2, ctx.csr_t, ctx.b2_param, ctx.w_refs = nbr, d2, csr_t, b2_param, w_refs
        return m

    @staticmethod
    def backward(ctx, dm):
        ab, wd, w2, pre2 = ctx.saved_tensors
        dm, dm_ld = _rows_ld(dm)
        N, Hp = ab.shape[0], ab.shape[1] // 2
        dev = ab.device
        dab = torch.empty_like(ab)
        tw = [_acc_target(q) for q in ctx.w_refs] if ctx.w_refs is not None else [None, None]
        w_acc = all(t is not None for t in tw)
        dwd = tw[0] if w_acc else torch.empty_like(wd)
        dw2 = tw[1] if w_acc else torch.empty_like(w2)
        dpre2 = torch.empty_like(pre2)
        L = hip.lib()
        ws_bytes = L.egnn_edge_bwd_workspace_bytes(N, Hp)
        ws = _workspace(ws_bytes, dev)
        tg = _acc_target(ctx.b2_param)
        db2 = tg if tg is not None else torch.empty(16, dtype=torch.float32, device=dev)
        timed("egnn_edge_bwd", N * 16 * Hp * 96,
              lambda: hip.check(L.egnn_edge_bwd_p(_ptr(ab), _ptr(wd), _ptr(w2), _ptr(ctx.nbr), _ptr(ctx.d2), _ptr(pre2),
                                                  _ptr(dm), dm_ld, _ptr(ctx.csr_t.rowptr), _ptr(ctx.csr_t.perm), N, Hp, _ptr(dab),
                                                  _ptr(dwd), _ptr(dw2), _ptr(dpre2), _ptr(db2), 1 if tg is not None else 0,
                                                  1 if w_acc else 0, _ptr(ws), ws_bytes, _stream(dev), ctx.products),
                                "egnn_edge_bwd"))
        return (dab, None if w_acc else dwd, None if w_acc else dw2, (None if tg is not None else db2), None, None, None, None,
                None)


class _EgnnFeats(torch.autograd.Function):

    @staticmethod
    def forward(ctx, feats, w_cat, b_cat, gamma, beta, eps, acc_params, w_refs=None):
        _require_gpu(feats, "egnn_feats")
        feats = _f32c(feats)
        R, C = feats.shape
        ctx.fold = gamma is None
        if ctx.fold:
            ab = mm_nt(feats, w_cat, bias=b_cat)
            ctx.save_for_backward(feats, w_cat)
            ctx.eps, ctx.acc, ctx.w_refs = 0.0, acc_params, w_refs
            ctx.set_materialize_grads(False)
            return ab, feats.view_as(feats), feats.view_as(feats)
        g, b = _f32c(gamma), _f32c(beta)
        normed = torch.empty_like(feats)
        hip.check(hip.lib().hg_layer_norm_fwd(_ptr(feats), _ptr(g), _ptr(b), R, C, float(eps), _ptr(normed),
                                              _stream(feats.device)), "hg_layer_norm_fwd")
        ab = mm_nt(feats, w_cat, bias=b_cat)
        ctx.save_for_backward(feats, w_cat, g)
        ctx.eps, ctx.acc, ctx.w_refs = float(eps), acc_params, w_refs
        ctx.set_materialize_grads(False)
        return ab, normed, feats.view_as(feats)

    @staticmethod
    def backward(ctx, d_ab, d_normed, d_res):
        if ctx.fold:
            feats, w_cat = ctx.saved_tensors
            gamma = None
            if d_normed is not None and d_res is not None:
                d_res = d_normed + d_res
            elif d_normed is not None:
                d_res = d_normed
            d_normed = None
        else:
            feats, w_cat, gamma = ctx.saved_tensors
        R, C = feats.shape
        dev = feats.device
        L = hip.lib()
        dgamma = dbeta = None
        if d_normed is not None:
            d_normed, dy_ld = _rows_ld(d_normed)
            add = _f32c(d_res) if d_res is not None else None
            dx = torch.empty_like(feats)
            ws_bytes = L.hg_layer_norm_bwd_workspace_bytes(R, C)
            ws = _workspace(ws_bytes, dev)
            tg = [_acc_target(p) for p in ctx.acc]
            in_place = all(t is not None for t in tg)
            small = tg if in_place else list(torch.empty((2, C), dtype=torch.float32, device=dev))
            hip.check(L.hg_layer_norm_bwd(_ptr(feats), _ptr(gamma), _ptr(d_normed), dy_ld, _ptr(add), R, C, ctx.eps, _ptr(dx),
                                          _ptr(small[0]), _ptr(small[1]), 1 if in_place else 0, _ptr(ws), ws_bytes,
                                          _stream(dev)), "hg_layer_norm_bwd")
            if not in_place:
                dgamma, dbeta = _hand_out(list(small), tg)
        elif ctx.fold:
            dx = _f32c(d_res) if d_res is not None else None
        else:
            dx = _f32c(d_res).clone() if d_res is not None else None
        dw = db = None
        if d_ab is not None:
            d_ab = _f32c(d_ab)
            if dx is None:
                dx = mm_nn(d_ab, w_cat)
            elif ctx.fold:
                dx = mm_nn(d_ab, w_cat, d=dx)
            else:
                dx = mm_nn(d_ab, w_cat, d=dx, out=dx)
            tw = [_acc_target(q) for q in ctx.w_refs] if ctx.w_refs is not None else [None, None]
            if ctx.needs_input_grad[1]:
                if tw[0] is not None:
                    if USE_X6 and R >= X6_WGRAD_ROWS and gemm_supported(d_ab, feats, True, False):
                        gemm(d_ab, feats, trans_a=True, trans_b=False, d=tw[0], out=tw[0])
                    elif not _wgrad_deferred(d_ab, feats, 1.0, tw[0]):
                        tw[0].addmm_(d_ab.t(), feats)
                elif USE_X6 and R >= X6_WGRAD_ROWS and gemm_supported(d_ab, feats, True, False):
                    dw = gemm(d_ab, feats, trans_a=True, trans_b=False)
                else:
                    dw = d_ab.t() @ feats
            if ctx.needs_input_grad[2]:
                if tw[1] is not None:
                    half = d_ab.shape[1] // 2
                    colsum(d_ab[:, :half], into=tw[1][:half])
                    db = None
                else:
                    db = colsum(d_ab)
        return dx, dw, db, dgamma, dbeta, None, None, None


def egnn_feats(feats, w_cat, b_cat, norm):
    if norm is None:
        return _EgnnFeats.apply(feats, w_cat, b_cat, None, None, 0.0, (), (w_cat, b_cat))
    _note_acc(norm.weight, norm.bias)
    return _EgnnFeats.apply(feats, w_cat, b_cat, norm.weight, norm.bias, norm.eps, (norm.weight, norm.bias), (w_cat, b_cat))


class _EgnnPackWeights(torch.autograd.Function):

    @staticmethod
    def forward(ctx, w1, b1, w2, Hp, acc_params):
        _require_gpu(w1, "egnn_pack_weights")
        w1, b1, w2 = _f32c(w1), _f32c(b1), _f32c(w2)
        H, in_ld = w1.shape
        C = (in_ld - 1) // 2
        dev = w1.device
        w_cat = torch.empty((2 * Hp, C), dtype=torch.float32, device=dev)
        b_cat = torch.empty(2 * Hp, dtype=torch.float32, device=dev)
        wd = torch.empty(Hp, dtype=torch.float32, device=dev)
        w2p = torch.empty((16, Hp), dtype=torch.float32, device=dev)
        hip.check(hip.lib().egnn_pack_weights_fwd(_ptr(w1), _ptr(b1), _ptr(w2), H, Hp, C, _ptr(w_cat), _ptr(b_cat),
                                                  _ptr(wd), _ptr(w2p), _stream(dev)), "egnn_pack_weights_fwd")
        ctx.dims = (H, Hp, C)
        ctx.acc = acc_params
        return w_cat, b_cat, wd, w2p

    @staticmethod
    def backward(ctx, dw_cat, db_cat, dwd, dw2p):
        H, Hp, C = ctx.dims
        dev = dw_cat.device
        tg = [_acc_target(p) for p in ctx.acc]
        in_place = all(t is not None for t in tg)
        if in_place:
            dw1, db1, dw2 = tg
        else:
            dw1 = torch.empty((H, 2 * C + 1), dtype=torch.float32, device=dev)
            db1 = torch.empty(H, dtype=torch.float32, device=dev)
            dw2 = torch.empty((16, H), dtype=torch.float32, device=dev)
        hip.check(hip.lib().egnn_pack_weights_bwd(_ptr(_f32c(dw_cat)), _ptr(_f32c(db_cat)), _ptr(_f32c(dwd)),
                                                  _ptr(_f32c(dw2p)), H, Hp, C, _ptr(dw1), _ptr(db1), _ptr(dw2),
                                                  1 if in_place else 0, _stream(dev)), "egnn_pack_weights_bwd")
        if in_place:
            return None, None, None, None, None
        return (*_hand_out([dw1, db1, dw2], tg), None, None)


def egnn_pack_weights(w1, b1, w2, Hp):
    if torch.is_grad_enabled():
        for w in (w1, b1, w2):
            if w.requires_grad and w.is_leaf:
                (LINEAR_PARAMS if w.dim() == 2 else ACC_PARAMS)[id(w)] = w
    res = _EgnnPackWeights.apply(w1, b1, w2, Hp, (w1, b1, w2))
    if not (DEFER_PACK_BWD and _DEFER["active"] and torch.is_grad_enabled() and any(t.requires_grad for t in res)):
        return res
    shapes = [(t.shape[0], t.shape[1]) if t.dim() == 2 else (1, t.shape[0]) for t in res]
    accs = [_merged_acc(sh, res[0].device).view(t.shape) for sh, t in zip(shapes, res)]
    leaves = []
    for t, a in zip(res, accs):
        leaf = t.detach().requires_grad_()
        leaf._eqh_transient = True
        leaf._eqh_gbuf = a
        leaves.append(leaf)
    _DEFER["merged"].append((list(res), accs))
    return tuple(leaves)


def egnn_edge(ab, wd, w2, b2, nbr, d2, csr_t: CSR):
    _note_acc(b2)
    return _EgnnEdge.apply(ab, wd, w2, b2, nbr, d2, csr_t, b2, (wd, w2))


NODE_WGRAD_BLOCKS = not os.environ.get("EQH_NO_NODE_WGRAD_BLOCKS")
DEFER_PACK_BWD = not os.environ.get("EQH_NO_DEFER_PACK")


class _EgnnNodeMlp(torch.autograd.Function):

    @staticmethod
    def forward(ctx, normed, m_i, res, w0, b0, w3, b3, gamma=None, beta=None, eps=0.0):
        from .panel import _products, conv_panel, panel_pack, panel_planes
        _require_gpu(normed, "egnn_node_mlp")
        ctx.products = _products()
        ctx.fold = gamma is not None
        normed, m_i = _f32c(normed), _f32c(m_i)
        res = normed if ctx.fold else _f32c(res)
        N, C = normed.shape
        dev = normed.device
        need_grad = any(ctx.needs_input_grad)
        items = [(w0[:C], True), (w0[C:], True), (w3, True)]
        if need_grad:
            items += [(w3[:, :C], False), (w3[:, C:], False), (w0, False, C + 32)]
        imgs = panel_pack(items, planes=panel_planes())
        node_in = torch.empty((N, C + 16), dtype=torch.float32, device=dev)
        hpre = torch.empty((N, 2 * C), dtype=torch.float32, device=dev)
        hid = torch.empty_like(hpre)
        out = torch.empty((N, C), dtype=torch.float32, device=dev)
        ln = dict(g0=_f32c(gamma), be0=_f32c(beta), eps=float(eps)) if ctx.fold else {}
        timed("k_node_f", 2 * N * ((C + 16) * 2 * C + 2 * C * C), lambda: conv_panel(
            hip.HG_EGNN_NODE_F, N, C, dev, in0=normed, in1=m_i, in2=res, w0=imgs[0], w1=imgs[1], w2=imgs[2], b0=b0, bias_out=b3,
            out0=node_in, out1=hpre, out2=hid, out3=out, **ln))
        if need_grad:
            if ctx.fold:
                ctx.save_for_backward(w0, b0, w3, b3, node_in, hpre, hid, m_i, normed, ln["g0"])
                ctx.ln = (gamma, beta, float(eps))
            else:
                ctx.save_for_backward(w0, b0, w3, b3, node_in, hpre, hid, m_i)
            ctx.imgs = imgs[3:]
        return out

    @staticmethod
    @backward_as_forward
    def backward(ctx, dout):
        from .panel import conv_panel, conv_panel_slab
        from .grads import _linear_weight_grad
        if ctx.fold:
            w0, b0, w3, b3, node_in, hpre, hid, m_i, feats, g0 = ctx.saved_tensors
        else:
            w0, b0, w3, b3, node_in, hpre, hid, m_i = ctx.saved_tensors
        N, C = hid.shape[0], hid.shape[1] // 2
        dev = dout.device
        dout, ld = _rows_ld(dout)
        dpre = torch.empty_like(hpre)
        dgam = dbet = None
        if ctx.fold:
            dfeats = torch.empty((N, C), dtype=torch.float32, device=dev)
            dm = torch.empty((N, 16), dtype=torch.float32, device=dev)
            p_gamma, p_beta, eps = ctx.ln
            tg = [_acc_target(p_gamma), _acc_target(p_beta)]
            acc = all(t is not None for t in tg)
            small = tg if acc else list(torch.empty((2, C), dtype=torch.float32, device=dev))
            junk = torch.empty(C, dtype=torch.float32, device=dev)
            timed("k_node_b", 2 * N * (2 * C * C + 2 * C * (C + 16)), lambda: conv_panel(
                hip.HG_EGNN_NODE_B, N, C, dev, eps=eps, accumulate=acc, in0=dout, ld0=ld, in1=hpre, w0=ctx.imgs[0], w1=ctx.imgs[1],
                w2=ctx.imgs[2], out0=dpre, out1=dfeats, out2=dm, in3=feats, g0=g0, slab=conv_panel_slab(N, C, dev), dbias=junk,
                dgamma=small[0], dbeta=small[1]))
            if not acc:
                dgam, dbet = small[0], small[1]
        else:
            dnode_in = torch.empty_like(node_in)
            timed("k_node_b", 2 * N * (2 * C * C + 2 * C * (C + 16)), lambda: conv_panel(
                hip.HG_EGNN_NODE_B, N, C, dev, in0=dout, ld0=ld, in1=hpre, w0=ctx.imgs[0], w1=ctx.imgs[1], w2=ctx.imgs[2], out0=dpre,
                out1=dnode_in))
        dout_c = dout if ld == C else dout.contiguous()
        dw3 = dw0 = None
        blocks = NODE_WGRAD_BLOCKS and _acc_target(w3) is not None and _acc_target(w0) is not None and C % 64 == 0
        if blocks:
            if ctx.needs_input_grad[5]:
                for c0 in (0, C):
                    _linear_weight_grad(w3, c0, c0 + C, dout_c, hid[:, c0:c0 + C])
            if ctx.needs_input_grad[3]:
                for r0 in (0, C):
                    _linear_weight_grad(w0, 0, C, dpre[:, r0:r0 + C], node_in[:, :C], r0, r0 + C)
                _linear_weight_grad(w0, C, C + 16, dpre, m_i)
        else:
            dw3 = _linear_weight_grad(w3, None, None, dout_c, hid) if ctx.needs_input_grad[5] else None
            dw0 = _linear_weight_grad(w0, None, None, dpre, node_in) if ctx.needs_input_grad[3] else None
        db3 = colsum(dout_c, into=_acc_target(b3)) if ctx.needs_input_grad[6] else None
        db0 = colsum(dpre, into=_acc_target(b0)) if ctx.needs_input_grad[4] else None
        if ctx.fold:
            return dfeats, dm, None, dw0, db0, dw3, db3, dgam, dbet, None
        return dnode_in[:, :C], dnode_in[:, C:], dout, dw0, db0, dw3, db3, None, None, None


def egnn_node_mlp_supported(normed, m_i, lin0, lin3) -> bool:
    from .panel import panel_supported
    C = normed.shape[-1]
    return (normed.is_cuda and normed.dim() == 2 and normed.dtype == torch.float32 and panel_supported(C) and m_i.shape[-1] == 16
            and tuple(lin0.weight.shape) == (2 * C, C + 16) and tuple(lin3.weight.shape) == (C, 2 * C) and normed.shape[0] > 0)


def egnn_node_mlp(normed, m_i, res, lin0, lin3):
    if torch.is_grad_enabled():
        for w in (lin0.weight, lin3.weight):
            if w.requires_grad and w.is_leaf:
                LINEAR_PARAMS[id(w)] = w
    _note_acc(lin0.bias, lin3.bias)
    return _EgnnNodeMlp.apply(normed, m_i, res, lin0.weight, lin0.bias, lin3.weight, lin3.bias)


NODE_LN_FOLD = not os.environ.get("EQH_NO_NODE_LN_FOLD")


def egnn_node_mlp_ln(feats, m_i, lin0, lin3, norm):
    if torch.is_grad_enabled():
        for w in (lin0.weight, lin3.weight):
            if w.requires_grad and w.is_leaf:
                LINEAR_PARAMS[id(w)] = w
    _note_acc(lin0.bias, lin3.bias, norm.weight, norm.bias)
    return _EgnnNodeMlp.apply(feats, m_i, None, lin0.weight, lin0.bias, lin3.weight, lin3.bias, norm.weight, norm.bias, norm.eps)
```

include/equihgnn_hip.h:

```cpp
#ifndef EQUIHGNN_HIP_H
#define EQUIHGNN_HIP_H

#include <stddef.h>
#include <stdint.h>

#ifdef __cplusplus
extern "C" {
#endif

#define EQH_OK 0
#define EQH_ERR_ARG (-1)
#define EQH_ERR_ALIGN (-2)
#define EQH_ERR_RANGE (-3)
#define EQH_ERR_LAUNCH (-4)

int eqh_version(void);
const char* eqh_error_string(int code);

int eqh_adam_step(float* param, float* grad, float* exp_avg, float* exp_avg_sq, int64_t n,
                  const float* lr, float beta1, float beta2, float eps, float weight_decay, float grad_scale,
                  void* state, int32_t zero_grad, float* zero_also, int64_t zero_also_n, void* stream);
int eqh_copy_many(int32_t count, const float* const* src, float* const* dst, const int64_t* n, void* stream);
int eqh_add_many(int32_t count, const float* const* src, float* const* dst, const int64_t* n,
                 float* zero_also, int64_t zero_also_n, void* stream);
size_t eqh_grad_sumsq_workspace_bytes(int64_t n);
int eqh_grad_sumsq(const float* grad, int64_t n, void* partials, void* stream);
int eqh_adam_step_clip(float* param, float* grad, float* exp_avg, float* exp_avg_sq, int64_t n,
                       const float* lr, float beta1, float beta2, float eps, float weight_decay, float grad_scale,
                       void* state, int32_t zero_grad, float* zero_also, int64_t zero_also_n,
                       const void* partials, float max_norm, float* readout, void* stream);
int eqh_adam_step_ema(float* param, float* grad, float* exp_avg, float* exp_avg_sq, int64_t n,
                      const float* lr, float beta1, float beta2, float eps, float weight_decay, float grad_scale,
                      void* state, int32_t zero_grad, float* zero_also, int64_t zero_also_n,
                      float* ema, float decay, int32_t warmup, void* stream);
int eqh_adam_step_clip_ema(float* param, float* grad, float* exp_avg, float* exp_avg_sq, int64_t n,
                           const float* lr, float beta1, float beta2, float eps, float weight_decay, float grad_scale,
                           void* state, int32_t zero_grad, float* zero_also, int64_t zero_also_n,
                           const void* partials, float max_norm, float* readout,
                           float* ema, float decay, int32_t warmup, void* stream);
int eqh_swap_f32(float* a, float* b, int64_t n, void* stream);
int eqh_mse_fwd_bwd(const float* pred, const float* target, int32_t n, float* loss, float* grad, void* stream);
int eqh_smooth_l1_fwd_bwd(const float* pred, const float* target, int32_t n, float beta, float scale, float* loss,
                          float* grad, void* stream);
int eqh_bootstrap_update(const float* pred, const float* target, int64_t n, float scale, int32_t copies, int64_t seed,
                         int64_t position0, void* acc, void* stream);
int eqh_loss_accumulate(const float* loss, void* acc, void* stream);
int eqh_bootstrap_weights_host(int64_t seed, int64_t position0, int64_t n, int32_t copies, int32_t* out);

int eqh_defer_begin(void* stream);
int eqh_defer_flush(void* stream);

typedef struct HgGemmProblem {
    const float* a;
    int64_t lda;
    const float* b;
    int64_t ldb;
    const float* d;
    int64_t ldd;
    const float* bias;
    float* c;
    int64_t ldc;
    int64_t m;
    int32_t n, k;
    int32_t trans_a, trans_b, relu;
    float alpha, beta;
    const int64_t* drop_seed;
    float drop_p;
    int32_t mean_rows;
    const void* b_packed;
} HgGemmProblem;
size_t hg_gemm_x6_workspace_bytes(int32_t n_problems, const HgGemmProblem* problems, int32_t tile);
int32_t hg_gemm_x6_choose_tile(int32_t n_problems, const HgGemmProblem* problems, int32_t with_workspace);
int hg_gemm_x6_batch(int32_t n_problems, const HgGemmProblem* problems, int32_t tile, void* workspace, size_t workspace_bytes,
                     void* stream);
int hg_gemm_bf16_batch(int32_t n_problems, const HgGemmProblem* problems, int32_t tile, int32_t products, void* workspace,
                       size_t workspace_bytes, void* stream);

typedef struct HgSmallMM {
    const float* a;
    int64_t a_rs, a_cs;
    const float* b;
    int64_t b_rs, b_cs;
    float* c;
    int64_t ldc;
    const float* u;
    const float* v;
    const float* x;
    const float* z;
    float* y;
    float* w;
    int32_t m, n, k;
    float alpha;
    int32_t accumulate_c, accumulate_y;
} HgSmallMM;
int hg_small_mm_batch(int32_t n_problems, const HgSmallMM* problems, void* stream);

typedef struct {
    const float* w;
    int64_t ld;
    void* dst;
    int32_t K, N, trans, kstep0, ksteps_total;
    int32_t n_valid;
    int32_t k_major;
    int32_t planes;
} HgPanelPack;
size_t hg_panel_pack_bytes(int32_t K, int32_t N);
size_t hg_panel_pack_bytes_p(int32_t K, int32_t N, int32_t planes);
int hg_panel_pack(int32_t n_items, const HgPanelPack* items, void* stream);
int hg_panel_gemm_f32(const float* a, int64_t lda, int64_t rows, int32_t C, const void* wpack, float alpha,
                      const float* d, int64_t ldd, float beta, const float* bias, int32_t relu, float* c, int64_t ldc,
                      void* stream);
int hg_panel_gemm_f32_p(const float* a, int64_t lda, int64_t rows, int32_t C, const void* wpack, float alpha,
                        const float* d, int64_t ldd, float beta, const float* bias, int32_t relu, float* c, int64_t ldc,
                        int32_t products, int32_t planes, void* stream);
int hg_panel_stream_supported(int32_t K, int32_t N);
int hg_panel_stream_gemm_f32(const float* a, int64_t lda, int64_t rows, int32_t K, int32_t N, const void* wpack, float alpha,
                             const float* d, int64_t ldd, float beta, const float* bias, int32_t relu, float* c, int64_t ldc,
                             void* stream);
int hg_panel_stream_gemm_f32_p(const float* a, int64_t lda, int64_t rows, int32_t K, int32_t N, const void* wpack, float alpha,
                               const float* d, int64_t ldd, float beta, const float* bias, int32_t relu, float* c, int64_t ldc,
                               int32_t products, int32_t planes, void* stream);

enum { HG_CONV_F1 = 1, HG_CONV_F2 = 2, HG_CONV_F3 = 3, HG_CONV_B3 = 4, HG_CONV_B1 = 5, HG_EGNN_NODE_F = 6, HG_EGNN_NODE_B = 7 };
typedef struct {
    int64_t rows;
    int32_t C;
    float eps, scale;
    int32_t relu, acc_first, tail, accumulate;
    const float *in0, *in1, *in2, *in3;
    int64_t ld0;
    const int32_t *rowptr, *col;
    const float* wq;
    const void *w0, *w1, *w2, *w3;
    const float *b0, *g0, *be0, *b1, *g1, *be1, *bias_out;
    float *out0, *out1, *out2, *out3, *out4, *out5;
    float *slab, *slab2, *acc_out;
    float *dbias, *dgamma, *dbeta, *dbias2, *dgamma2, *dbeta2;
    const float *g_inc, *be_inc;
    float eps_inc;
    float* out6;
    int32_t* signal;
    int32_t products, planes;
} HgConvPanel;
size_t hg_conv_panel_slab_bytes(int64_t rows, int32_t C);
int hg_conv_panel(int32_t stage, const HgConvPanel* args, void* stream);
typedef struct {
    float p_inc; const int64_t* seed_inc; const int32_t* perm;
    float p;     const int64_t* seed;
} HgConvDrop;
int hg_conv_panel_drop(int32_t stage, const HgConvPanel* args, const HgConvDrop* drop, void* stream);
typedef struct {
    float p_inc; const int64_t* seed_inc; const int32_t* perm;
    float p3;    const int64_t* seed3;
    float p_x;   const int64_t* seed_x;
    float p1;    const int64_t* seed1;
} HgConvStackDrop;
int hg_conv_stack_drop(int32_t stage, const HgConvPanel* args, const HgConvStackDrop* drop, void* stream);
int hg_conv_stack_drop_f3_launches(int32_t C, int32_t products);
typedef struct {
    const float* a;
    int64_t lda, rows;
    int32_t C, n;
    const void* w[3];
    const float* bias[3];
    const float* rw[3];
    const float* d[3];
    int64_t ldd[3];
    float* out[3];
    int64_t ldo[3];
    int32_t products, planes;
} HgPanelMulti;
int hg_panel_multi(const HgPanelMulti* args, void* stream);
typedef struct {
    const float* a[3];
    int64_t lda[3];
    int64_t rows;
    int32_t C, n;
    const void* w[3];
    const float* d;
    int64_t ldd;
    float* out;
    int64_t ldo;
    int32_t products, planes;
} HgPanelSum;
int hg_panel_sum(const HgPanelSum* args, void* stream);
int32_t hg_panel_waves(void);

typedef struct {
    int64_t B, n_mols;
    const int64_t* idx;
    const int64_t *node_off, *he_off, *inc_off;
    const int64_t* x;
    const float* pos;
    const int64_t *v, *e, *edge_attr, *e_order;
    const float* y;
    int64_t PN, PM, PZ;
    int32_t padded;
    int64_t* out_x;
    float* out_pos;
    int64_t *out_edge_index0, *out_edge_index1, *out_edge_attr, *out_n_e, *out_e_order, *out_batch;
    float* out_y;
    int64_t* out_counts;
} HbCollate;
int hb_collate(const HbCollate* args);

typedef struct {
    int64_t B, n_mols;
    const int64_t* idx;
    const int64_t *node_off, *edge_off;
    const int64_t* x;
    const int64_t *src, *dst, *edge_attr;
    int64_t F;
    const float* y;
    int64_t PN, PE;
    int32_t padded;
    int64_t *out_x, *out_edge_index, *out_edge_attr, *out_batch;
    float* out_y;
    int64_t* out_counts;
} GbCollate;
int gb_collate(const GbCollate* args);

typedef struct {
    int64_t B, n_mols;
    const int64_t* idx;
    const int64_t *node_off, *he_off, *inc_off;
    const int64_t* x;
    const float* pos;
    const int64_t *v, *e, *edge_attr, *e_order;
    const float* y;
    int64_t PN, PM, PZ;
    int32_t padded;
    int64_t* out_x;
    float* out_pos;
    int64_t *out_edge_index0, *out_edge_index1, *out_edge_attr, *out_n_e, *out_e_order, *out_batch;
    float* out_y;
    int64_t* out_counts;
    void* workspace;
    int64_t workspace_bytes;
} HbCollateDev;
int hb_collate_dev(const HbCollateDev* args, void* stream);
int64_t hb_collate_dev_workspace_bytes(int64_t B);

typedef struct {
    int64_t B, n_mols;
    const int64_t* idx;
    const int64_t *node_off, *edge_off;
    const int64_t* x;
    const int64_t *src, *dst, *edge_attr;
    int64_t F;
    const float* y;
    int64_t PN, PE;
    int32_t padded;
    int64_t *out_x, *out_edge_index, *out_edge_attr, *out_batch;
    float* out_y;
    int64_t* out_counts;
    void* workspace;
    int64_t workspace_bytes;
} GbCollateDev;
int gb_collate_dev(const GbCollateDev* args, void* stream);
int64_t gb_collate_dev_workspace_bytes(int64_t B);

int eqh_stamp(void* slot, void* stream);
int64_t eqh_wall_clock_khz(void);
int eqh_clock_probe(void* out, int32_t spin_us, void* stream);
int eqh_signal_post(int32_t* counter, void* stream);
int eqh_signal_wait(const int32_t* counter, int32_t target, int32_t timeout_us, void* stream);
int eqh_accumulate(const float* src, float* dst, int64_t n, void* stream);
int eqh_event_create(void** event);
int eqh_event_record(void* event, void* stream);
int eqh_event_wait(void* event, void* stream);
int eqh_event_destroy(void* event);

size_t hg_csr_build_workspace_bytes(int64_t nnz, int64_t n_rows);
int hg_csr_build(const int64_t* key, const int64_t* other, int64_t nnz, int64_t n_rows,
                 int32_t col_div, int32_t* rowptr, int32_t* perm, int32_t* col,
                 void* workspace, size_t workspace_bytes, void* stream);
int hg_csr_build_i32(const int32_t* key, const int64_t* other, int64_t nnz, int64_t n_rows, int32_t col_div,
                     int32_t* rowptr, int32_t* perm, int32_t* col, void* workspace, size_t workspace_bytes,
                     void* stream);
int hg_csr_build_i32_counted(const int32_t* key, const int64_t* other, int64_t nnz, int64_t n_rows, int32_t col_div,
                             int32_t* rowptr, int32_t* perm, int32_t* col, int32_t* counts, void* workspace,
                             size_t workspace_bytes, void* stream);
int hg_index_aux(const int64_t* vertex, const int64_t* edges, int64_t nnz, const int64_t* batch,
                 int64_t n_nodes, int64_t n_edges, const int32_t* rowptr_v, const int32_t* rowptr_e,
                 int32_t* v32, int32_t* e32, int32_t* batch32, float* has_v, float* has_e,
                 const int32_t* col_v, const int32_t* col_e, float* ew_v, float* ew_e, int32_t* zero_buf, int64_t zero_n,
                 void* stream);
size_t hg_csr_build_batch_workspace_bytes(int32_t n, const int64_t* nnz, const int64_t* n_rows);
int hg_csr_build_batch(int32_t n, const int64_t* const* key, const int64_t* const* other, const int64_t* nnz,
                       const int64_t* n_rows, const int32_t* col_div, int32_t* const* rowptr,
                       int32_t* const* perm, int32_t* const* col, void* workspace, size_t workspace_bytes,
                       void* stream);

int hg_segment_reduce_f32(const float* src, const int32_t* idx, const int32_t* rowptr,
                          const int32_t* src_wptr, float* out, int64_t n_out_rows, int32_t C,
                          int32_t mean, void* stream);
int hg_entry_weights(const int32_t* idx, const int32_t* wptr, int64_t nnz, float* w, void* stream);
int hg_segment_reduce_w_f32(const float* src, const int32_t* idx, const int32_t* rowptr, const float* entry_w, float* out,
                            int64_t n_out_rows, int32_t C, void* stream);

int hg_pool_pair_fwd(const float* x, const int32_t* x_rowptr, const int32_t* x_perm, int64_t n_x, const float* e,
                     const int32_t* e_rowptr, const int32_t* e_perm, const int64_t* e_order, int64_t n_e, float* out,
                     int64_t B, int32_t C, void* stream);
int hg_pool_pair_bwd(const float* dout, const int32_t* x_mol, int64_t n_x, const int32_t* e_mol, const int64_t* e_order,
                     int64_t n_e, float* dx, float* de, int64_t B, int32_t C, void* stream);

int hg_embed_sum_fwd(const int64_t* x, const float* table, const int32_t* off_host, int32_t F,
                     int64_t N, int32_t C, int64_t table_rows, float* out, void* stream);

size_t hg_embed_sum_bwd_workspace_bytes(int64_t N, int32_t C, int64_t table_rows);
int hg_embed_sum_bwd(const int64_t* x, const float* dout, const int32_t* off_host, int32_t F,
                     int64_t N, int32_t C, int64_t table_rows, float* dtable, int32_t accumulate,
                     void* workspace, size_t workspace_bytes, void* stream);

int geo_knn(const float* pos, int64_t N, int32_t k, int32_t mode, int32_t* nbr, float* dist,
            void* stream);
int geo_knn_counted(const float* pos, int64_t N, int32_t k, int32_t mode, int32_t* nbr, float* dist, int32_t* counts,
                    void* stream);

int egnn_edge_fwd(const float* ab, const float* wd, const float* w2, const float* b2,
                  const int32_t* nbr, const float* d2, int64_t N, int32_t Hp, float* m, float* pre2,
                  void* stream);
size_t egnn_edge_bwd_workspace_bytes(int64_t N, int32_t Hp);
int egnn_edge_bwd(const float* ab, const float* wd, const float* w2, const int32_t* nbr,
                  const float* d2, const float* pre2, const float* dm, int64_t dm_ld, const int32_t* t_rowptr,
                  const int32_t* t_perm, int64_t N, int32_t Hp, float* dab, float* dwd, float* dw2,
                  float* dpre2, float* db2, int32_t db2_accumulate, int32_t dw_accumulate, void* workspace,
                  size_t workspace_bytes, void* stream);
int egnn_edge_fwd_p(const float* ab, const float* wd, const float* w2, const float* b2,
                    const int32_t* nbr, const float* d2, int64_t N, int32_t Hp, float* m, float* pre2,
                    void* stream, int32_t products);
int egnn_edge_bwd_p(const float* ab, const float* wd, const float* w2, const int32_t* nbr,
                    const float* d2, const float* pre2, const float* dm, int64_t dm_ld, const int32_t* t_rowptr,
                    const int32_t* t_perm, int64_t N, int32_t Hp, float* dab, float* dwd, float* dw2,
                    float* dpre2, float* db2, int32_t db2_accumulate, int32_t dw_accumulate, void* workspace,
                    size_t workspace_bytes, void* stream, int32_t products);

int hg_rowgemm_fwd(const float* z, const float* w, const int32_t* rowptr, const int32_t* perm,
                   int64_t R, int32_t Kd, int32_t L, float* out, int32_t accumulate, void* stream);
int hg_rowgemm_bwd(const float* z, const float* w, const float* dout, const int32_t* rowptr,
                   const int32_t* perm, int64_t R, int32_t Kd, int32_t L, float* dz,
                   int32_t accumulate_dz, float* dw, void* stream);
int hg_rowgemm_bias_supported(int32_t Kd, int32_t L);
int hg_rowgemm_fwd_bias(const float* z, const float* w, const int32_t* rowptr, const int32_t* perm, int64_t R, int32_t Kd,
                        int32_t L, float* out, int32_t accumulate, const float* rowbias, const float* coef, int32_t MB,
                        int32_t z_factored, void* stream);
int hg_rowgemm_bwd_bias(const float* z, const float* w, const float* dout, const int32_t* rowptr, const int32_t* perm,
                        int64_t R, int32_t Kd, int32_t L, float* dz, int32_t accumulate_dz, float* dw, const float* coef,
                        int32_t MB, float* drowbias, int32_t z_factored, void* stream);

int hg_incidence_ln_reduce_fwd(const float* pa, const float* qb, const int32_t* ia, const int32_t* ib,
                               const int32_t* rowptr, const int32_t* perm, const float* gamma,
                               const float* beta, int64_t n_rows, int32_t C, int32_t mean, float eps,
                               float* out, void* stream);
int hg_incidence_ln_reduce_fwd_col(const float* pa, const float* qb, const int32_t* rowptr, const int32_t* col,
                                   int32_t row_is_a, const float* gamma, const float* beta, int64_t n_rows, int32_t C,
                                   int32_t mean, float eps, float* out, void* stream);
size_t hg_incidence_ln_reduce_bwd_workspace_bytes(int64_t n_a_rows, int32_t C);
int hg_incidence_ln_reduce_bwd(const float* pa, const float* qb, const int32_t* ia, const int32_t* ib,
                               const int32_t* a_rowptr, const int32_t* a_perm, int64_t n_a_rows,
                               const int32_t* b_rowptr, const int32_t* b_perm, int64_t n_b_rows,
                               const int32_t* okey, const int32_t* orowptr, const float* ds,
                               const float* gamma, int32_t C, int32_t mean, float eps, float* dpa,
                               float* dqb, float* dgamma, int32_t accumulate, void* workspace,
                               size_t workspace_bytes, void* stream);

int hg_bias_relu_ln_fwd(const float* h, const float* bias, const float* gamma, const float* beta,
                        int64_t n_rows, int32_t C, float eps, float* out, void* stream);
size_t hg_bias_relu_ln_bwd_workspace_bytes(int64_t n_rows, int32_t C);
int hg_bias_relu_ln_bwd(const float* h, const float* bias, const float* gamma, const float* dy,
                        int64_t n_rows, int32_t C, float eps, float* dh, float* dbias, float* dgamma,
                        float* dbeta, int32_t accumulate, void* workspace, size_t workspace_bytes,
                        void* stream);
int hg_bias_relu_ln_fwd_ex(const float* h, float h_scale, const float* pre_add, const float* bias, const float* gamma,
                           const float* beta, int64_t n_rows, int32_t C, float eps, float* out, void* stream);
int hg_bias_relu_ln_bwd_ex(const float* h, float h_scale, const float* pre_add, const float* bias, const float* gamma,
                           const float* dy, int64_t n_rows, int32_t C, float eps, float* dh, float* dbias, float* dgamma,
                           float* dbeta, int32_t accumulate, void* workspace, size_t workspace_bytes, float* acc_out,
                           int32_t acc_first, void* stream);

int hg_gather_ln_reduce_fwd(const float* h, const float* bias, const float* gamma, const float* beta,
                            const int32_t* rowptr, const int32_t* col, int64_t n_rows, int32_t C, int32_t mean,
                            float eps, float* out, void* stream);
size_t hg_gather_ln_reduce_bwd_workspace_bytes(int64_t n_src_rows, int32_t C);
int hg_gather_ln_reduce_bwd(const float* h, const float* bias, const float* gamma, const float* dout,
                            const int32_t* t_rowptr, const int32_t* t_col, const float* t_w, int64_t n_src_rows,
                            int32_t C, float eps, float* dh, float* dbias, float* dgamma, float* dbeta,
                            int32_t accumulate, void* workspace, size_t workspace_bytes, void* stream);

int hg_bias_relu_ln_drop_fwd(const float* h, float h_scale, const float* pre_add, const float* bias, const float* gamma,
                             const float* beta, int64_t n_rows, int32_t C, float eps, float p, const int64_t* seed,
                             float* out, void* stream);
size_t hg_bias_relu_ln_drop_bwd_workspace_bytes(int64_t n_rows, int32_t C);
int hg_bias_relu_ln_drop_bwd(const float* h, float h_scale, const float* pre_add, const float* bias, const float* gamma,
                             const float* dy, int64_t n_rows, int32_t C, float eps, float p, const int64_t* seed, float* dh,
                             float* dbias, float* dgamma, float* dbeta, int32_t accumulate, void* workspace,
                             size_t workspace_bytes, float* acc_out, int32_t acc_first, void* stream);
int hg_gather_ln_reduce_drop_fwd(const float* h, const float* bias, const float* gamma, const float* beta,
                                 const int32_t* rowptr, const int32_t* col, int64_t n_rows, int32_t C, int32_t mean,
                                 float eps, float p, const int64_t* seed, float* out, void* stream);
size_t hg_gather_ln_reduce_drop_bwd_workspace_bytes(int64_t n_src_rows, int32_t C);
int hg_gather_ln_reduce_drop_bwd(const float* h, const float* bias, const float* gamma, const float* dout,
                                 const int32_t* t_rowptr, const int32_t* t_col, const float* t_w, int64_t n_src_rows,
                                 int32_t C, float eps, float p, const int64_t* seed, float* dh, float* dbias, float* dgamma,
                                 float* dbeta, int32_t accumulate, void* workspace, size_t workspace_bytes, void* stream);
int hg_incidence_ln_reduce_drop_fwd(const float* pa, const float* qb, const int32_t* ia, const int32_t* ib,
                                    const int32_t* rowptr, const int32_t* perm, const float* gamma, const float* beta,
                                    int64_t n_rows, int32_t C, int32_t mean, float eps, float p, const int64_t* seed,
                                    float* out, void* stream);
int hg_incidence_ln_reduce_drop_fwd_col(const float* pa, const float* qb, const int32_t* rowptr, const int32_t* col,
                                        const int32_t* perm, int32_t row_is_a, const float* gamma, const float* beta,
                                        int64_t n_rows, int32_t C, int32_t mean, float eps, float p, const int64_t* seed,
                                        float* out, void* stream);
size_t hg_incidence_ln_reduce_drop_bwd_workspace_bytes(int64_t n_a_rows, int32_t C);
int hg_incidence_ln_reduce_drop_bwd(const float* pa, const float* qb, const int32_t* ia, const int32_t* ib,
                                    const int32_t* a_rowptr, const int32_t* a_perm, int64_t n_a_rows,
                                    const int32_t* b_rowptr, const int32_t* b_perm, int64_t n_b_rows, const int32_t* okey,
                                    const int32_t* orowptr, const float* ds, const float* gamma, int32_t C, int32_t mean,
                                    float eps, float p, const int64_t* seed, float* dpa, float* dqb, float* dgamma,
                                    float* dbeta, int32_t accumulate, void* workspace, size_t workspace_bytes, void* stream);

size_t hg_batch_norm_rows_workspace_bytes(int64_t R, int32_t C);
int hg_batch_norm_rows_fwd(const float* x, const float* row_mask, const float* gamma, const float* beta,
                           float* running_mean, float* running_var, int64_t* num_batches_tracked, float momentum, float eps,
                           int64_t R, int32_t C, float* y, float* save_mean, float* save_rstd, int32_t relu, void* workspace,
                           size_t workspace_bytes, void* stream);
int hg_batch_norm_rows_bwd(const float* x, const float* dy, const float* row_mask, const float* gamma,
                           const float* save_mean, const float* save_rstd, int64_t R, int32_t C, float* dx, float* dgamma,
                           float* dbeta, const float* beta, int32_t relu, void* workspace, size_t workspace_bytes, void* stream);

int hg_layer_norm_fwd(const float* x, const float* gamma, const float* beta, int64_t n_rows, int32_t C,
                      float eps, float* out, void* stream);
size_t hg_layer_norm_bwd_workspace_bytes(int64_t n_rows, int32_t C);
int hg_layer_norm_bwd(const float* x, const float* gamma, const float* dy, int64_t dy_ld, const float* add,
                      int64_t n_rows, int32_t C, float eps, float* dx, float* dgamma, float* dbeta, int32_t accumulate,
                      void* workspace, size_t workspace_bytes, void* stream);

int64_t geo_knn_grid_max_points(void);
size_t geo_knn_grid_workspace_bytes(int64_t N);
int geo_knn_grid(const float* pos, int64_t N, int32_t k, int32_t mode, const int32_t* n_box, int32_t* nbr,
                 float* dist, void* workspace, size_t workspace_bytes, void* stream);

int faf_attn_sum_fwd(const float* attn, const float* x, int64_t N, int32_t K, int32_t H, int32_t D, float* out,
                     void* stream);
int faf_attn_sum_bwd(const float* attn, const float* x, const float* dout, int64_t N, int32_t K, int32_t H, int32_t D,
                     float* dx, float* dattn, void* stream);
int faf_attn_gather_sum_fwd(const float* attn, const float* x, int64_t x_ld, const int32_t* nbr, int64_t N, int32_t K,
                            int32_t H, int32_t D, float* out, void* stream);
int faf_attn_gather_sum_bwd(const float* attn, const float* x, int64_t x_ld, const int32_t* nbr, const float* dout,
                            const int32_t* rowptr, const int32_t* perm, int64_t N, int64_t NS, int32_t K, int32_t H,
                            int32_t D, float* dattn, float* dx, void* stream);

size_t faf_moments_workspace_bytes(int64_t N);
int faf_centre_mix_fwd(const float* geo, const float* logit, const float* row_mask, int64_t N, float* out, float* aux,
                       void* workspace, size_t workspace_bytes, void* stream);
int faf_centre_mix_bwd(const float* dout, const float* geo, const float* logit, const float* row_mask, const float* aux,
                       int64_t N, float* dgeo, float* dlogit, void* workspace, size_t workspace_bytes, void* stream);
int faf_cloud_frame_fwd(const float* x, const float* row_mask, int64_t N, float* y, float* aux, void* workspace,
                        size_t workspace_bytes, void* stream);
int faf_cloud_frame_bwd(const float* dy, const float* row_mask, const float* aux, int64_t N, float* dx, void* workspace,
                        size_t workspace_bytes, void* stream);
int faf_edge_frame_fwd(const float* geo, const float* gj, const uint8_t* mask, int64_t N, int32_t K, float* y, float* d2,
                       float* V, void* stream);
int faf_edge_frame_bwd(const float* geo, const float* gj, const uint8_t* mask, const float* V, const float* dy,
                       const float* dd2, int64_t N, int32_t K, float* dgeo, float* dgj, void* stream);
int faf_attn_logits_fwd(const float* qa, const float* qan, const float* le, const uint8_t* mask, int64_t N, int32_t K,
                        int32_t H, float p, const int64_t* seed, float* prob, float* attn, void* stream);
int faf_dropout_add(const float* x, const float* res, int64_t n, float p, const int64_t* seed, float* out, void* stream);
int faf_ln_rowdot_fwd(const float* x, const float* gamma, const float* beta, const float* U, const float* cb, int64_t R,
                      int32_t C, int32_t J, float eps, float* out, float* le, void* stream);
size_t faf_ln_rowdot_bwd_workspace_bytes(int64_t R, int32_t C, int32_t J);
int faf_ln_rowdot_bwd(const float* x, const float* gamma, const float* beta, const float* U, const float* dy, int64_t dy_ld,
                      const float* dle, const float* add, int64_t R, int32_t C, int32_t J, float eps, float* dx, float* dgamma,
                      float* dbeta, int32_t accumulate, float* dU, void* workspace, size_t workspace_bytes, void* stream);
int faf_edge_logit_weights_fwd(const float* W, int64_t ldw, const float* b, const float* we, int32_t H, int32_t deh, int32_t de,
                               float* u, float* c, void* stream);
int faf_edge_logit_weights_bwd(const float* W, int64_t ldw, const float* b, const float* we, const float* du, const float* dc,
                               int32_t H, int32_t deh, int32_t de, float* dW, int64_t lddw, float* db, float* dwe,
                               int32_t acc_w, int32_t acc_b, int32_t acc_e, void* stream);
int faf_attn_logits_bwd(const float* prob, const float* dattn, const uint8_t* mask, int64_t N, int32_t K, int32_t H, float p,
                        const int64_t* seed, float* dqa, float* dqan, float* dle, void* stream);

int eqf_edge_geometry(const float* pos, const int32_t* nbr, const float* dist, int64_t N, int32_t K, float radius,
                      float* rhat, float* maskf, float* mean_w, float* mean_w_rhat, float* dmat, void* stream);

int eqf_pool3(const float* src, const float* w3, int64_t N, int32_t K, int32_t C, int32_t backward, float* dst, void* stream);

int eqf_rms_norm_fwd(const float* x, const float* g, int64_t n_rows, int32_t C, float scale, float eps, float* out,
                     void* stream);
size_t eqf_rms_norm_bwd_workspace_bytes(int64_t n_rows, int32_t C);
int eqf_rms_norm_bwd(const float* x, const float* g, const float* dy, int64_t n_rows, int32_t C, float scale,
                     float eps, float* dx, float* dg, int32_t accumulate, void* workspace, size_t workspace_bytes,
                     void* stream);

int eqf_attn_pool_fwd(const float* me, const float* edge, const float* mask, const float* w_logit, const float* wv,
                      int64_t N, int32_t K, int32_t D, int32_t v_off, int32_t V, float scale, float slope, float* out,
                      float* attn, void* stream);
size_t eqf_attn_pool_bwd_workspace_bytes(int64_t N);
int eqf_attn_pool_bwd(const float* me, const float* edge, const float* mask, const float* w_logit, const float* wv,
                      const float* attn, const float* dout, int64_t N, int32_t K, int32_t D, int32_t v_off, int32_t V,
                      float scale, float slope, float* dme, float* dedge, float* dw_logit, float* dwv,
                      int32_t accumulate, void* workspace, size_t workspace_bytes, void* stream);

int eqf_radial_trunk_fwd(const float* dist, const float* const* params, int64_t E, int32_t M, float eps,
                         float* out, void* stream);
size_t eqf_radial_trunk_bwd_workspace_bytes(int64_t E);
int eqf_radial_trunk_bwd(const float* dist, const float* const* params, const float* dh, int64_t E, int32_t M,
                         float eps, float* const* dparams, int32_t accumulate, void* workspace,
                         size_t workspace_bytes, void* stream);

int hg_readout_mse_supported(int32_t C, int32_t H);
size_t hg_readout_mse_workspace_bytes(int32_t n_graphs, int32_t C, int32_t H);
int hg_readout_mse_f32(const float* x, const int32_t* rowptr, int32_t n_graphs, int32_t n_real, int32_t C,
                       int32_t H, const float* const* weights, float eps, const float* target, float* y,
                       float* loss, float* dx, float* const* dweights, int32_t accumulate, void* workspace,
                       size_t workspace_bytes, int32_t* state, void* stream);
int hg_readout_mse_drop_f32(const float* x, const int32_t* rowptr, int32_t n_graphs, int32_t n_real, int32_t C,
                            int32_t H, const float* const* weights, float eps, const float* target, float* y,
                            float* loss, float* dx, float* const* dweights, int32_t accumulate, void* workspace,
                            size_t workspace_bytes, int32_t* state, float p_x, float p_h, const int64_t* seed_x,
                            const int64_t* seed_h1, const int64_t* seed_h2, void* stream);
int hg_readout_sl1_f32(const float* x, const int32_t* rowptr, int32_t n_graphs, int32_t n_real, int32_t C,
                       int32_t H, const float* const* weights, float eps, const float* target, float* y,
                       float* loss, float* dx, float* const* dweights, int32_t accumulate, void* workspace,
                       size_t workspace_bytes, int32_t* state, float beta, float scale, void* stream);
int hg_readout_sl1_drop_f32(const float* x, const int32_t* rowptr, int32_t n_graphs, int32_t n_real, int32_t C,
                            int32_t H, const float* const* weights, float eps, const float* target, float* y,
                            float* loss, float* dx, float* const* dweights, int32_t accumulate, void* workspace,
                            size_t workspace_bytes, int32_t* state, float p_x, float p_h, const int64_t* seed_x,
                            const int64_t* seed_h1, const int64_t* seed_h2, float beta, float scale, void* stream);

int hg_readout_pair_mse_supported(int32_t C, int32_t H);
size_t hg_readout_pair_mse_workspace_bytes(int32_t n_graphs, int32_t C, int32_t H);
int hg_readout_pair_mse_f32(const float* x, const int32_t* rowptr, const float* e, const int32_t* e_rowptr,
                            const int32_t* e_perm, const int64_t* e_order, int32_t n_e, int32_t n_graphs, int32_t n_real,
                            int32_t C, int32_t H, const float* const* weights, float eps, const float* target, float* y,
                            float* loss, float* dx, float* de, float* const* dweights, int32_t accumulate, void* workspace,
                            size_t workspace_bytes, int32_t* state, void* stream);
int hg_readout_pair_mse_drop_f32(const float* x, const int32_t* rowptr, const float* e, const int32_t* e_rowptr,
                                 const int32_t* e_perm, const int64_t* e_order, int32_t n_e, int32_t n_graphs,
                                 int32_t n_real, int32_t C, int32_t H, const float* const* weights, float eps,
                                 const float* target, float* y, float* loss, float* dx, float* de,
                                 float* const* dweights, int32_t accumulate, void* workspace, size_t workspace_bytes,
                                 int32_t* state, float p_x, float p_h, const int64_t* seed_x, const int64_t* seed_e,
                                 const int64_t* seed_h1, const int64_t* seed_h2, void* stream);
int hg_readout_pair_sl1_f32(const float* x, const int32_t* rowptr, const float* e, const int32_t* e_rowptr,
                            const int32_t* e_perm, const int64_t* e_order, int32_t n_e, int32_t n_graphs, int32_t n_real,
                            int32_t C, int32_t H, const float* const* weights, float eps, const float* target, float* y,
                            float* loss, float* dx, float* de, float* const* dweights, int32_t accumulate, void* workspace,
                            size_t workspace_bytes, int32_t* state, float beta, float scale, void* stream);
int hg_readout_pair_sl1_drop_f32(const float* x, const int32_t* rowptr, const float* e, const int32_t* e_rowptr,
                                 const int32_t* e_perm, const int64_t* e_order, int32_t n_e, int32_t n_graphs,
                                 int32_t n_real, int32_t C, int32_t H, const float* const* weights, float eps,
                                 const float* target, float* y, float* loss, float* dx, float* de,
                                 float* const* dweights, int32_t accumulate, void* workspace, size_t workspace_bytes,
                                 int32_t* state, float p_x, float p_h, const int64_t* seed_x, const int64_t* seed_e,
                                 const int64_t* seed_h1, const int64_t* seed_h2, float beta, float scale, void* stream);

int faf_swiglu_dropout_fwd(const float* pre, int64_t R, int32_t H, float p, const int64_t* seed, float* out,
                           void* stream);
int faf_swiglu_dropout_bwd(const float* pre, const float* dout, int64_t R, int32_t H, float p, const int64_t* seed,
                           float* dpre, void* stream);
int faf_dropout_mean_fwd(const float* x, int64_t R, int32_t F, int32_t C, float p, const int64_t* seed, float* out,
                         void* stream);
int faf_dropout_mean_bwd(const float* dout, int64_t R, int32_t F, int32_t C, float p, const int64_t* seed, float* dx,
                         void* stream);
size_t faf_dropout_mean_bwd_colsum_workspace_bytes(int64_t R, int32_t F, int32_t C);
int faf_dropout_mean_bwd_colsum(const float* dout, int64_t R, int32_t F, int32_t C, float p, const int64_t* seed, float* dx,
                                float* colsum, int32_t accumulate, void* workspace, size_t workspace_bytes, void* stream);
int faf_frame_pre_fwd(const float* y, const float* w3, const float* base, int64_t E, int32_t H, float* out, void* stream);
size_t faf_frame_pre_bwd_workspace_bytes(int64_t E, int32_t H);
int faf_frame_pre_bwd(const float* y, const float* w3, const float* dpre, int64_t E, int32_t H, float* dy, float* dbase,
                      float* dw3, int32_t accumulate, void* workspace, size_t workspace_bytes, void* stream);

int faf_frame_hidden_fwd(const float* y, const float* w3, const float* base, int64_t base_ld, const float* extra,
                         const float* wx, const float* gamma, const float* beta, int64_t E, float p, const int64_t* seed,
                         float eps, float* out, int32_t w_ld, void* stream);
size_t faf_frame_hidden_bwd_workspace_bytes(int64_t E);
int faf_frame_hidden_bwd(const float* y, const float* w3, const float* base, int64_t base_ld, const float* extra,
                         const float* wx, const float* gamma, const float* dhn, int64_t E, float p, const int64_t* seed,
                         float eps, float* dy, float* dbase, float* dwx, float* dextra, float* dw3, float* dgamma,
                         float* dbeta, int32_t accumulate, int32_t w_ld, void* workspace, size_t workspace_bytes,
                         void* stream);

int faf_rowdot_fwd(const float* x, const float* U, const float* bias, int64_t R, int32_t C, int32_t J, float* y, void* stream);
size_t faf_rowdot_bwd_workspace_bytes(int64_t R, int32_t C, int32_t J);
int faf_rowdot_bwd(const float* x, const float* U, const float* dy, const float* dx_add, int64_t R, int32_t C, int32_t J,
                   float* dx, float* dU, int32_t accumulate, void* workspace, size_t workspace_bytes, void* stream);

int faf_gate_fwd(const float* x, const float* w, const float* b, const float* res, int64_t R, int32_t C, float p,
                 const int64_t* seed, float* out, void* stream);
size_t faf_gate_bwd_workspace_bytes(int64_t R, int32_t C);
int faf_gate_bwd(const float* x, const float* w, const float* b, const float* dout, int64_t R, int32_t C, float p,
                 const int64_t* seed, float* dx, float* dw, float* db, int32_t accumulate, float* dx_colsum,
                 int32_t accumulate_colsum, void* workspace, size_t workspace_bytes, void* stream);

int faf_edge_hidden_fwd(const float* A, const float* B, const float* Cf, const int32_t* nbr, const float* gamma,
                        const float* beta, int64_t N, int32_t K, float p, const int64_t* seed, float eps, float* out,
                        void* stream);
size_t faf_edge_hidden_bwd_workspace_bytes(int64_t N);
int faf_edge_hidden_bwd(const float* A, const float* B, const float* Cf, const int32_t* nbr, const float* gamma,
                        const float* dhn, int64_t N, int32_t K, float p, const int64_t* seed, float eps, float* dpre, float* dA,
                        float* dgamma, float* dbeta, int32_t accumulate, void* workspace, size_t workspace_bytes, void* stream);

int eqh_permute_tiles_f32(const float* src, float* dst, int32_t nX, int32_t nY, int32_t nY_pad, int32_t nB, int64_t sY,
                          int64_t sB, int64_t dX, int64_t dB, void* stream);

int geo_eigh3(const float* a, int64_t B, float* w, float* v, void* stream);

size_t hg_wgrad_workspace_bytes(int64_t K, int32_t O, int32_t I);
int hg_wgrad_f32(const float* dy, const float* x, int64_t K, int32_t O, int32_t I, float alpha, float* dw,
                 int64_t ldw, int32_t accumulate, void* workspace, size_t workspace_bytes, void* stream);
size_t hg_wgrad_skinny_workspace_bytes(int64_t K, int32_t O, int32_t J);
int hg_wgrad_skinny_f32(const float* dy, int64_t ld_dy, const float* x, int64_t ld_x, int64_t K, int32_t O, int32_t J, float alpha,
                        float* dw, int64_t ldw, int32_t accumulate, void* workspace, size_t workspace_bytes, void* stream);
size_t hg_wgrad_batch_workspace_bytes(int32_t count, int32_t O, int32_t I);
int hg_wgrad_batch_f32(int32_t count, const float* const* dy, const float* const* x, const int64_t* K, int32_t O,
                       int32_t I, const float* alpha, float* const* dw, const int64_t* ldw, int32_t accumulate,
                       void* workspace, size_t workspace_bytes, void* stream,
                       const int64_t* ld_dy, const int64_t* ld_x);
int hg_wgrad_batch_bf16(int32_t count, const float* const* dy, const float* const* x, const int64_t* K, int32_t O,
                        int32_t I, const float* alpha, float* const* dw, const int64_t* ldw, int32_t accumulate,
                        void* workspace, size_t workspace_bytes, void* stream,
                        const int64_t* ld_dy, const int64_t* ld_x, int32_t products);
size_t hg_colsum_workspace_bytes(int64_t R, int32_t C);
int hg_colsum_f32(const float* x, const int32_t* rowptr, int32_t weight_mode, float scale, int64_t R, int32_t C,
                  int32_t accumulate, float* out, void* workspace, size_t workspace_bytes, void* stream);
int hg_residual_mix_f32(const float* x0, const float* bias, const int32_t* rowptr, int32_t weight_mode,
                        float alpha, int64_t R, int32_t C, float* out, void* stream);
size_t hg_colsum_batch_workspace_bytes(int32_t count, const int64_t* R, const int32_t* C);
int hg_colsum_batch_f32(int32_t count, const float* const* x, const int64_t* ld, const int32_t* const* rowptr,
                        const int32_t* weight_mode, const float* scale, const int64_t* R, const int32_t* C,
                        float* const* out, void* workspace, size_t workspace_bytes, void* stream);
int egnn_pack_weights_fwd(const float* w1, const float* b1, const float* w2, int32_t H, int32_t Hp,
                          int32_t C, float* w_cat, float* b_cat, float* wd, float* w2p, void* stream);
int egnn_pack_weights_bwd(const float* dw_cat, const float* db_cat, const float* dwd, const float* dw2p,
                          int32_t H, int32_t Hp, int32_t C, float* dw1, float* db1, float* dw2,
                          int32_t accumulate, void* stream);

int hg_edge_codes(const int64_t* edge_attr, int32_t F, const int32_t* off_host, int32_t T, const int32_t* eid,
                  int64_t nnz, int32_t* code, void* stream);
int hg_edge_msg_fwd(int32_t mode, const float* x, const float* tables, int32_t T, int32_t F, const int32_t* in_rowptr,
                    const int32_t* in_src, const int32_t* in_code, const int32_t* out_rowptr, const float* eps,
                    const float* root, int64_t N, int32_t C, float* out, void* stream);
size_t hg_edge_msg_bwd_workspace_bytes(int64_t N, int32_t C, int32_t T);
int hg_edge_msg_bwd(int32_t mode, const float* x, const float* tables, int32_t T, int32_t F, const int32_t* out_rowptr,
                    const int32_t* out_dst, const int32_t* out_code, const float* eps, const float* root,
                    const float* dout, int64_t N, int32_t C, float* dx, float* dtables, float* dextra,
                    int32_t accumulate, void* workspace, size_t workspace_bytes, void* stream);

int vis_radius_graph(const float* pos, const int32_t* batch, const int32_t* pool_rowptr, const int32_t* n_real,
                     const float* means, const float* betas, int64_t N, float cutoff, int32_t* slot, int32_t* cnt,
                     float* r, float* cut, float* rbf, float* sh, int32_t* src_start, int32_t* src_cnt,
                     int32_t* src_eid, void* stream);
int vis_nbr_fwd(const float* x, const float* W, const float* cut, const int32_t* slot, const int32_t* cnt, int64_t N,
                int32_t C, float* y, void* stream);
int vis_nbr_bwd(const float* x, const float* W, const float* cut, const int32_t* slot, const int32_t* cnt,
                const int32_t* src_start, const int32_t* src_cnt, const int32_t* src_eid, const float* dy, int64_t N,
                int32_t C, float* dx, float* dW, void* stream);
int vis_edge_embed_fwd(const float* x, const float* W, const int32_t* slot, const int32_t* cnt, int64_t N, int32_t C,
                       float* f, void* stream);
int vis_edge_embed_bwd(const float* x, const float* W, const int32_t* slot, const int32_t* cnt,
                       const int32_t* src_start, const int32_t* src_cnt, const int32_t* src_eid, const float* df,
                       int64_t N, int32_t C, float* dx, float* dW, void* stream);
int vis_attn_fwd(const float* q, const float* k, const float* v, const float* dkr, const float* dvr, const float* cut,
                 const int32_t* slot, const int32_t* cnt, int64_t N, int32_t C, float* u, float* xagg, float* pre,
                 void* stream);
int vis_attn_bwd(const float* q, const float* k, const float* v, const float* dkr, const float* dvr, const float* cut,
                 const float* pre, const int32_t* slot, const int32_t* cnt, const int32_t* src_start,
                 const int32_t* src_cnt, const int32_t* src_eid, const float* du, const float* dxagg, int64_t N,
                 int32_t C, float* dq, float* dk, float* dv, float* ddkr, float* ddvr, float* dpre, void* stream);
int vis_vec_fwd(const float* vec, const float* sr, const float* sh, const int32_t* slot, const int32_t* cnt, int64_t N,
                int32_t C, float* vo, void* stream);
int vis_vec_bwd(const float* vec, const float* sr, const float* sh, const int32_t* slot, const int32_t* cnt,
                const int32_t* src_start, const int32_t* src_cnt, const int32_t* src_eid, const float* dvo, int64_t N,
                int32_t C, float* dvec, float* dsr, void* stream);
int vis_edge_update_fwd(const float* wt, const float* ws, const float* fr, const float* sh, const int32_t* slot,
                        const int32_t* cnt, int64_t N, int32_t C, float* df, void* stream);
int vis_edge_update_bwd(const float* wt, const float* ws, const float* fr, const float* sh, const int32_t* slot,
                        const int32_t* cnt, const int32_t* src_start, const int32_t* src_cnt, const int32_t* src_eid,
                        const float* ddf, int64_t N, int32_t C, float* dwt, float* dws, float* dfr, void* stream);

int se3t_edge_basis(const float* pos, const int32_t* nbr, int64_t N, int32_t K, float radius, const float* qtab,
                    float* dist, float* maskf, float* meanw, float* basis, void* stream);
size_t se3t_pair_fwd_workspace_bytes(int64_t E, int32_t MO, int32_t O, int32_t pooled);
int se3t_pair_fwd(const float* h, const float* G, const float* GB, const float* coef, int32_t cstride,
                  const int32_t* rowptr, const int32_t* perm, int64_t N, int64_t E, int32_t MO, int32_t Q, int32_t O,
                  const float* meanw, int32_t K, float* out, int32_t accumulate, void* workspace, size_t workspace_bytes,
                  void* stream);
int se3t_pair_bwd(const float* h, const float* G, const float* coef, int32_t cstride, const int32_t* rowptr,
                  const int32_t* perm, int64_t N, int64_t E, int32_t MO, int32_t Q, int32_t O, const float* dout,
                  const float* meanw, int32_t K, float* dh, float* dG, float* dGB, void* stream);
int se3t_attn_fwd(const float* q, const float* kself, const float* kedge, const float* vself, const float* vedge,
                  const float* maskf, int64_t N, int32_t K, int32_t M, float scale, float* out, float* logits,
                  void* stream);
int se3t_attn_bwd(const float* q, const float* kself, const float* kedge, const float* vself, const float* vedge,
                  const float* logits, const float* dout, int64_t N, int32_t K, int32_t M, float scale, float* dq,
                  float* dkself, float* dkedge, float* dvself, float* dvedge, void* stream);
int se3t_norm_fwd(const float* x, const float* scale, int64_t R, int32_t M, int32_t C, float eps, float* out, void* stream);
size_t se3t_norm_bwd_workspace_bytes(int64_t R, int32_t C);
int se3t_norm_bwd(const float* x, const float* scale, const float* dy, int64_t R, int32_t M, int32_t C, float eps, float* dx,
                  float* dscale, void* workspace, size_t workspace_bytes, void* stream);

#ifdef __cplusplus
}
#endif
#endif
```

Measured before the change: 228,600 molecules/s.

## Skip padded hidden columns in EGNN edge backward with narrow tail tiles

Passes the live hidden width (hdim) into the edge backward so the recv and send kernels only run full 64-column tiles over live columns. A remainder of 16 or fewer columns is handled by a narrow scalar-per-lane tail path, and padded columns are zero-filled instead of computed. The send kernel now splits senders by edge count, using a wave-wide binary search over the transposed rowptr, in place of equal node chunks. This adds code paths and more complex grid sizing in exchange for less wasted work on padding and better load balance.

```diff
diff --git a/equihgnn_amd/csrc/egnn_edge.hip b/equihgnn_amd/csrc/egnn_edge.hip
--- a/equihgnn_amd/csrc/egnn_edge.hip
+++ b/equihgnn_amd/csrc/egnn_edge.hip
@@ -510,18 +510,173 @@
     return (dh0 + dh1) + (dh2 + dh3);
 }
 
+constexpr int NARROW_UNITS = 16, RECV_SPAN_MAX = 2, SEND_SPAN_MAX = 1;
+struct BwTiles {
+    int full, narrow, z0, span;
+    __host__ __device__ bool tail() const { return narrow || z0 >= 0; }
+};
+static inline BwTiles bw_tiles(int Hp, int h_live) {
+    const int live = (h_live + 63) >> 6, rem = h_live - 64 * (live - 1);
+    BwTiles t;
+    t.narrow = rem <= NARROW_UNITS ? 1 : 0;
+    t.full = live - t.narrow;
+    t.z0 = t.narrow ? 64 * t.full + NARROW_UNITS : 64 * live;
+    if (t.z0 >= Hp) t.z0 = -1;
+    t.span = 1;
+    return t;
+}
+static inline int bw_tail_items(const BwTiles& t, int chunks) { return t.tail() ? (chunks + t.span - 1) / t.span : 0; }
+static inline int bw_chunks_live(int64_t n_items, BwTiles& t, int span_max) {
+    int best = 0;
+    for (int span = 1; span <= (t.narrow ? span_max : 1); ++span) {
+        BwTiles u = t;
+        u.span = span;
+        int c = bw_chunks(n_items, u.full > 0 ? u.full : 1);
+        while (c > 1 && (int64_t)u.full * c + bw_tail_items(u, c) > BW_RESIDENT) --c;
+        if (c > best) best = c, t.span = span;
+    }
+    return best;
+}
+
+__device__ __forceinline__ void zero_columns(float* __restrict__ p, int64_t ld, int rows, int z0, int Hp, int lane) {
+    for (int row = 0; row < rows; ++row)
+        for (int c = z0 + lane; c < Hp; c += 64) p[(int64_t)row * ld + c] = 0.f;
+}
+
+struct RecvOps1 {
+    float4 pa, pt, dd;
+    float a, b0, b1, b2, b3;
+};
+
+__device__ __forceinline__ void recv_load1(RecvOps1& o, const float* __restrict__ ab, const float* __restrict__ d2,
+                                           const float* __restrict__ dpre2, const float* __restrict__ dpre2_t,
+                                           int node, int4 nb, int Hp, int k1, int r, int q) {
+    o.pa = *reinterpret_cast<const float4*>(dpre2 + (int64_t)node * 256 + r * MDIM + 4 * q);
+    o.pt = *reinterpret_cast<const float4*>(dpre2_t + (int64_t)node * 256 + r * KNB + 4 * q);
+    o.dd = *reinterpret_cast<const float4*>(d2 + (int64_t)node * KNB + 4 * q);
+    o.a = ab[(int64_t)node * 2 * Hp + k1];
+    o.b0 = ab[(int64_t)nb.x * 2 * Hp + Hp + k1];
+    o.b1 = ab[(int64_t)nb.y * 2 * Hp + Hp + k1];
+    o.b2 = ab[(int64_t)nb.z * 2 * Hp + Hp + k1];
+    o.b3 = ab[(int64_t)nb.w * 2 * Hp + Hp + k1];
+}
+
+template <int NP>
+__device__ __forceinline__ void recv_chunk16(float (*s_red)[64 * 20], const float* __restrict__ ab, const float* __restrict__ wd,
+                                             const float* __restrict__ w2, const int* __restrict__ nbr,
+                                             const float* __restrict__ d2, const float* __restrict__ dpre2,
+                                             const float* __restrict__ dpre2_t, float* __restrict__ dab,
+                                             float* __restrict__ slab_w2, float* __restrict__ slab_wd, int N, int Hp, int T,
+                                             int chunk, int chunk_nodes, int lane, int wave) {
+    const int r = lane & 15, q = lane >> 4;
+    const int base = chunk * chunk_nodes;
+    const int cnt = (N - base < chunk_nodes) ? (N - base) : chunk_nodes;
+    const int k1 = 64 * T + r;
+    const float w0 = w2[(4 * q + 0) * Hp + k1], w1 = w2[(4 * q + 1) * Hp + k1];
+    const float w2v = w2[(4 * q + 2) * Hp + k1], w3 = w2[(4 * q + 3) * Hp + k1];
+    const float wdc = wd[k1];
+    Planes4 wp = {};
+    if constexpr (NP != 6) wp = split_quad<edge_planes(NP)>(w0, w1, w2v, w3);
+    f32x4 aw = {0.f, 0.f, 0.f, 0.f};
+    float ad = 0.f;
+    const int4* __restrict__ nbr4 = reinterpret_cast<const int4*>(nbr);
+    const int last = cnt - 1;
+    auto clampn = [&](int x) { return base + (x < last ? x : last); };
+    auto one = [&](const RecvOps1& o, int node) {
+        f32x4 g = {0.f, 0.f, 0.f, 0.f};
+        Planes4 ptp = {};
+        if constexpr (NP == 6) {
+            g = mfma16(o.pa.x, w0, g);
+            g = mfma16(o.pa.y, w1, g);
+            g = mfma16(o.pa.z, w2v, g);
+            g = mfma16(o.pa.w, w3, g);
+        } else {
+            g = mfma16_planes<NP>(split_quad<edge_planes(NP)>(o.pa.x, o.pa.y, o.pa.z, o.pa.w), wp, g);
+            ptp = split_quad<edge_planes(NP)>(o.pt.x, o.pt.y, o.pt.z, o.pt.w);
+        }
+        float da = recv_column<NP>(o.a, wdc, o.dd, o.b0, o.b1, o.b2, o.b3, g, o.pt, ptp, ad, aw);
+        da += __shfl_xor(da, 16, 64);
+        da += __shfl_xor(da, 32, 64);
+        if (q == 0) dab[(int64_t)node * 2 * Hp + k1] = da;
+    };
+    if (wave < cnt) {
+        constexpr int U = NP == 3 ? 2 : 3;
+        int4 nb0 = nbr4[(int64_t)clampn(wave) * 4 + q], nb1 = nbr4[(int64_t)clampn(wave + WAVES) * 4 + q];
+        int4 nb2 = nbr4[(int64_t)clampn(wave + 2 * WAVES) * 4 + q];
+        for (int n = wave; n < cnt; n += U * WAVES) {
+            RecvOps1 o0, o1, o2;
+            recv_load1(o0, ab, d2, dpre2, dpre2_t, clampn(n), nb0, Hp, k1, r, q);
+            recv_load1(o1, ab, d2, dpre2, dpre2_t, clampn(n + WAVES), nb1, Hp, k1, r, q);
+            if constexpr (U > 2) recv_load1(o2, ab, d2, dpre2, dpre2_t, clampn(n + 2 * WAVES), nb2, Hp, k1, r, q);
+            nb0 = nbr4[(int64_t)clampn(n + U * WAVES) * 4 + q];
+            nb1 = nbr4[(int64_t)clampn(n + (U + 1) * WAVES) * 4 + q];
+            if constexpr (U > 2) nb2 = nbr4[(int64_t)clampn(n + (U + 2) * WAVES) * 4 + q];
+            one(o0, base + n);
+            if (n + WAVES < cnt) one(o1, base + n + WAVES);
+            if constexpr (U > 2)
+                if (n + 2 * WAVES < cnt) one(o2, base + n + 2 * WAVES);
+        }
+    }
+    ad += __shfl_xor(ad, 16, 64);
+    ad += __shfl_xor(ad, 32, 64);
+    if (wave > 0) {
+        float* p = &s_red[wave - 1][lane * 20];
+        *reinterpret_cast<f32x4*>(p) = aw;
+        p[4] = ad;
+    }
+    __syncthreads();
+    if (wave == 0) {
+#pragma unroll
+        for (int w = 0; w < WAVES - 1; ++w) {
+            const float* p = &s_red[w][lane * 20];
+            aw += *reinterpret_cast<const f32x4*>(p);
+            ad += p[4];
+        }
+        float* __restrict__ sw = slab_w2 + (int64_t)chunk * (MDIM + 1) * Hp;
+#pragma unroll
+        for (int g = 0; g < 4; ++g) sw[(4 * q + g) * Hp + k1] = aw[g];
+        if (q == 0) slab_wd[(int64_t)chunk * (MDIM + 1) * Hp + k1] = ad;
+    }
+    __syncthreads();
+}
+
+template <int NP>
+__device__ __forceinline__ void recv_tail(float (*s_red)[64 * 20], const float* __restrict__ ab, const float* __restrict__ wd,
+                                          const float* __restrict__ w2, const int* __restrict__ nbr, const float* __restrict__ d2,
+                                          const float* __restrict__ dpre2, const float* __restrict__ dpre2_t,
+                                          float* __restrict__ dab, float* __restrict__ slab_w2, float* __restrict__ slab_wd, int N,
+                                          int Hp, BwTiles bt, int first, int chunks, int chunk_nodes, int lane, int wave) {
+    for (int chunk = first; chunk < first + bt.span && chunk < chunks; ++chunk) {
+        if (bt.narrow)
+            recv_chunk16<NP>(s_red, ab, wd, w2, nbr, d2, dpre2, dpre2_t, dab, slab_w2, slab_wd, N, Hp, bt.full, chunk, chunk_nodes,
+                             lane, wave);
+        if (bt.z0 >= 0) {
+            const int base = chunk * chunk_nodes;
+            const int cnt = (N - base < chunk_nodes) ? (N - base) : chunk_nodes;
+            for (int n = wave; n < cnt; n += WAVES) zero_columns(dab + (int64_t)(base + n) * 2 * Hp, 0, 1, bt.z0, Hp, lane);
+            if (wave == 0) zero_columns(slab_w2 + (int64_t)chunk * (MDIM + 1) * Hp, Hp, MDIM + 1, bt.z0, Hp, lane);
+        }
+    }
+}
+
 template <int NP>
 __global__ void __launch_bounds__(THREADS)
 k_edge_bwd_recv(const float* __restrict__ ab, const float* __restrict__ wd, const float* __restrict__ w2,
                 const int* __restrict__ nbr, const float* __restrict__ d2, const float* __restrict__ dpre2,
                 const float* __restrict__ dpre2_t, float* __restrict__ dab, float* __restrict__ slab_w2,
-                float* __restrict__ slab_wd, int N, int Hp, int tiles, int chunk_nodes, int n_items, int remap) {
+                float* __restrict__ slab_wd, int N, int Hp, BwTiles bt, int chunks, int chunk_nodes, int n_items, int remap) {
     __shared__ __attribute__((aligned(16))) float s_red[WAVES - 1][64 * 20];
     const int lane = threadIdx.x & 63;
     const int wave = __builtin_amdgcn_readfirstlane(threadIdx.x >> 6);
     const int r = lane & 15, q = lane >> 4;
     const int item = xcd_item((int)blockIdx.x, (int)gridDim.x, n_items, remap);
     if (item < 0) return;
+    if (item >= bt.full * chunks) {
+        recv_tail<NP>(s_red, ab, wd, w2, nbr, d2, dpre2, dpre2_t, dab, slab_w2, slab_wd, N, Hp, bt,
+                      (item - bt.full * chunks) * bt.span, chunks, chunk_nodes, lane, wave);
+        return;
+    }
+    const int tiles = bt.full;
     const int T = item % tiles, chunk = item / tiles;
     const int base = chunk * chunk_nodes;
     const int cnt = (N - base < chunk_nodes) ? (N - base) : chunk_nodes;
@@ -623,15 +778,37 @@
 
 constexpr int SEND_LD = 68;
 
+__device__ __forceinline__ int rowptr_lower_bound(const int* __restrict__ t_rowptr, int N, int64_t x, int lane) {
+    int lo = 0, hi = N;
+    while (hi > lo) {
+        const int step = (hi - lo + 63) >> 6;
+        const int64_t idx = (int64_t)lo + (int64_t)lane * step;
+        const bool below = idx < hi && (int64_t)t_rowptr[idx] < x;
+        const int f = __popcll(__ballot(below));
+        if (f == 0) return lo;
+        const int new_hi = (f < 64 && (int64_t)lo + (int64_t)f * step < hi) ? lo + f * step : hi;
+        lo = lo + (f - 1) * step + 1;
+        hi = new_hi;
+    }
+    return lo;
+}
+
+template <int NU> struct UnitsOf { using type = float4; };
+template <> struct UnitsOf<1> { using type = float; };
+
+template <int NU>
 struct SendOps {
+    using V = typename UnitsOf<NU>::type;
     float4 pa;
-    float4 a0, a1, a2, a3;
-    float4 b0, b1, b2, b3;
+    V a0, a1, a2, a3;
+    V b0, b1, b2, b3;
     float dd0, dd1, dd2, dd3;
 };
 
-__device__ __forceinline__ void send_load(SendOps& o, const float* __restrict__ ab,
+template <int NU>
+__device__ __forceinline__ void send_load(SendOps<NU>& o, const float* __restrict__ ab,
                                           const float* __restrict__ dpre2, int4 rc, int Hp, int k4, int q) {
+    using V = typename UnitsOf<NU>::type;
     o.pa = *reinterpret_cast<const float4*>(dpre2 + (int64_t)rc.x * MDIM + 4 * q);
     const int e0 = __shfl(rc.x, 4 * q + 0, 64), e1 = __shfl(rc.x, 4 * q + 1, 64);
     const int e2 = __shfl(rc.x, 4 * q + 2, 64), e3 = __shfl(rc.x, 4 * q + 3, 64);
@@ -641,14 +818,20 @@
     o.dd1 = __int_as_float(__shfl(rc.z, 4 * q + 1, 64));
     o.dd2 = __int_as_float(__shfl(rc.z, 4 * q + 2, 64));
     o.dd3 = __int_as_float(__shfl(rc.z, 4 * q + 3, 64));
-    o.a0 = *reinterpret_cast<const float4*>(ab + (int64_t)(e0 >> 4) * 2 * Hp + k4);
-    o.a1 = *reinterpret_cast<const float4*>(ab + (int64_t)(e1 >> 4) * 2 * Hp + k4);
-    o.a2 = *reinterpret_cast<const float4*>(ab + (int64_t)(e2 >> 4) * 2 * Hp + k4);
-    o.a3 = *reinterpret_cast<const float4*>(ab + (int64_t)(e3 >> 4) * 2 * Hp + k4);
-    o.b0 = *reinterpret_cast<const float4*>(ab + (int64_t)j0 * 2 * Hp + Hp + k4);
-    o.b1 = *reinterpret_cast<const float4*>(ab + (int64_t)j1 * 2 * Hp + Hp + k4);
-    o.b2 = *reinterpret_cast<const float4*>(ab + (int64_t)j2 * 2 * Hp + Hp + k4);
-    o.b3 = *reinterpret_cast<const float4*>(ab + (int64_t)j3 * 2 * Hp + Hp + k4);
+    o.a0 = *reinterpret_cast<const V*>(ab + (int64_t)(e0 >> 4) * 2 * Hp + k4);
+    o.a1 = *reinterpret_cast<const V*>(ab + (int64_t)(e1 >> 4) * 2 * Hp + k4);
+    o.a2 = *reinterpret_cast<const V*>(ab + (int64_t)(e2 >> 4) * 2 * Hp + k4);
+    o.a3 = *reinterpret_cast<const V*>(ab + (int64_t)(e3 >> 4) * 2 * Hp + k4);
+    o.b0 = *reinterpret_cast<const V*>(ab + (int64_t)j0 * 2 * Hp + Hp + k4);
+    o.b1 = *reinterpret_cast<const V*>(ab + (int64_t)j1 * 2 * Hp + Hp + k4);
+    o.b2 = *reinterpret_cast<const V*>(ab + (int64_t)j2 * 2 * Hp + Hp + k4);
+    o.b3 = *reinterpret_cast<const V*>(ab + (int64_t)j3 * 2 * Hp + Hp + k4);
+}
+
+__device__ __forceinline__ float send_row(float wdc, float dd, float a, float b, float gk) {
+    float ds;
+    silu_grad(fmaf(wdc, dd, a + b), &ds);
+    return gk * ds;
 }
 
 __device__ __forceinline__ float4 send_row(const float4& wd4, float dd, const float4& a4, const float4& b4,
@@ -662,39 +845,39 @@
     return dh;
 }
 
-template <int NP>
-__global__ void __launch_bounds__(THREADS)
-k_edge_bwd_send(const float* __restrict__ ab, const float* __restrict__ wd, const float* __restrict__ w2,
-                const float* __restrict__ dpre2, const int* __restrict__ t_rowptr, const int4* __restrict__ rec,
-                float* __restrict__ dab, int N, int Hp, int tiles, int chunk_senders, int n_items, int remap) {
-    __shared__ __attribute__((aligned(16))) float s_tile[WAVES][KNB * SEND_LD];
-    const int lane = threadIdx.x & 63;
-    const int wave = __builtin_amdgcn_readfirstlane(threadIdx.x >> 6);
+__device__ __forceinline__ void send_share(const int* __restrict__ t_rowptr, int N, int g, int W, int lane, int& s_beg, int& s_end) {
+    const int64_t E = t_rowptr[N];
+    s_beg = __builtin_amdgcn_readfirstlane(rowptr_lower_bound(t_rowptr, N, (int64_t)g * E / W, lane));
+    s_end = g + 1 == W ? N : __builtin_amdgcn_readfirstlane(rowptr_lower_bound(t_rowptr, N, (int64_t)(g + 1) * E / W, lane));
+}
+
+template <int NP, int NU>
+__device__ __forceinline__ void send_range(float* __restrict__ tile, const float* __restrict__ ab, const float* __restrict__ wd,
+                                           const float* __restrict__ w2, const float* __restrict__ dpre2,
+                                           const int* __restrict__ t_rowptr, const int4* __restrict__ rec,
+                                           float* __restrict__ dab, int N, int Hp, int T, int s_beg, int s_end, int lane) {
+    using V = typename UnitsOf<NU>::type;
     const int r = lane & 15, q = lane >> 4;
-    const int item = xcd_item((int)blockIdx.x, (int)gridDim.x, n_items, remap);
-    if (item < 0) return;
-    const int T = item % tiles, chunk = item / tiles;
-    const int k4 = 64 * T + 4 * r;
-    const int c_beg = chunk * chunk_senders;
-    const int c_cnt = (N - c_beg < chunk_senders) ? (N - c_beg) : chunk_senders;
-    const int per = (c_cnt + WAVES - 1) / WAVES;
-    const int s_beg = c_beg + ((wave * per < c_cnt) ? wave * per : c_cnt);
-    const int s_end = c_beg + (((wave + 1) * per < c_cnt) ? (wave + 1) * per : c_cnt);
+    const int k4 = 64 * T + NU * r;
+    const bool owner = NU == 4 || lane < NARROW_UNITS;
     if (s_beg >= s_end) return;
     const int p_beg = t_rowptr[s_beg], p_end = t_rowptr[s_end];
     float* drow = dab + Hp + 64 * T + lane;
     if (p_beg == p_end) {
-        for (int sj = s_beg; sj < s_end; ++sj) drow[(int64_t)sj * 2 * Hp] = 0.f;
+        if (owner)
+            for (int sj = s_beg; sj < s_end; ++sj) drow[(int64_t)sj * 2 * Hp] = 0.f;
         return;
     }
-    const float4 w0 = *reinterpret_cast<const float4*>(w2 + (4 * q + 0) * Hp + k4);
-    const float4 w1 = *reinterpret_cast<const float4*>(w2 + (4 * q + 1) * Hp + k4);
-    const float4 w2v = *reinterpret_cast<const float4*>(w2 + (4 * q + 2) * Hp + k4);
-    const float4 w3 = *reinterpret_cast<const float4*>(w2 + (4 * q + 3) * Hp + k4);
-    const float4 wd4 = *reinterpret_cast<const float4*>(wd + k4);
+    const V w0 = *reinterpret_cast<const V*>(w2 + (4 * q + 0) * Hp + k4);
+    const V w1 = *reinterpret_cast<const V*>(w2 + (4 * q + 1) * Hp + k4);
+    const V w2v = *reinterpret_cast<const V*>(w2 + (4 * q + 2) * Hp + k4);
+    const V w3 = *reinterpret_cast<const V*>(w2 + (4 * q + 3) * Hp + k4);
+    const V wd4 = *reinterpret_cast<const V*>(wd + k4);
     Planes4 wp0 = {}, wp1 = {}, wp2 = {}, wp3 = {};
-    if constexpr (NP != 6) w2_planes<NP>(w0, w1, w2v, w3, wp0, wp1, wp2, wp3);
-    float* tile = s_tile[wave];
+    if constexpr (NP != 6) {
+        if constexpr (NU == 4) w2_planes<NP>(w0, w1, w2v, w3, wp0, wp1, wp2, wp3);
+        else wp0 = split_quad<edge_planes(NP)>(w0, w1, w2v, w3);
+    }
     int rp_base = s_beg;
     int rp = t_rowptr[((rp_base + lane < N) ? rp_base + lane : N - 1) + 1];
     int cur = s_beg;
@@ -703,18 +886,18 @@
     const int p_last = p_end - 1;
     auto pos = [&](int p) { return (p + r < p_last) ? p + r : p_last; };
     int4 rc_next = rec[pos(p_beg)];
-    SendOps nx;
-    send_load(nx, ab, dpre2, rc_next, Hp, k4, q);
+    SendOps<NU> nx;
+    send_load<NU>(nx, ab, dpre2, rc_next, Hp, k4, q);
     rc_next = rec[pos(p_beg + KNB)];
     for (int p0 = p_beg; p0 < p_end; p0 += KNB) {
-        const SendOps cur_ops = nx;
-        send_load(nx, ab, dpre2, rc_next, Hp, k4, q);
+        const SendOps<NU> cur_ops = nx;
+        send_load<NU>(nx, ab, dpre2, rc_next, Hp, k4, q);
         rc_next = rec[pos(p0 + 2 * KNB)];
         __builtin_amdgcn_sched_barrier(0);
         const bool live_r = p0 + r < p_end;
         const float4 pa = live_r ? cur_ops.pa : make_float4(0.f, 0.f, 0.f, 0.f);
 #ifdef EDGE_ABLATE
-        {
+        if constexpr (NU == 4) {
             run += (pa.x + cur_ops.dd0) + ((cur_ops.a0.x + cur_ops.a1.y) + (cur_ops.a2.z + cur_ops.a3.w)) +
                    ((cur_ops.b0.x + cur_ops.b1.y) + (cur_ops.b2.z + cur_ops.b3.w));
             if ((p0 & 255) == 0) drow[(int64_t)cur * 2 * Hp] = run;
@@ -722,30 +905,46 @@
         }
 #endif
         f32x4 g0 = {0.f, 0.f, 0.f, 0.f}, g1 = g0, g2 = g0, g3 = g0;
-        if constexpr (NP == 6) {
-            g0 = mfma16(pa.x, w0.x, g0); g1 = mfma16(pa.x, w0.y, g1); g2 = mfma16(pa.x, w0.z, g2); g3 = mfma16(pa.x, w0.w, g3);
-            g0 = mfma16(pa.y, w1.x, g0); g1 = mfma16(pa.y, w1.y, g1); g2 = mfma16(pa.y, w1.z, g2); g3 = mfma16(pa.y, w1.w, g3);
-            g0 = mfma16(pa.z, w2v.x, g0); g1 = mfma16(pa.z, w2v.y, g1); g2 = mfma16(pa.z, w2v.z, g2); g3 = mfma16(pa.z, w2v.w, g3);
-            g0 = mfma16(pa.w, w3.x, g0); g1 = mfma16(pa.w, w3.y, g1); g2 = mfma16(pa.w, w3.z, g2); g3 = mfma16(pa.w, w3.w, g3);
+        if constexpr (NU == 4) {
+            if constexpr (NP == 6) {
+                g0 = mfma16(pa.x, w0.x, g0); g1 = mfma16(pa.x, w0.y, g1); g2 = mfma16(pa.x, w0.z, g2); g3 = mfma16(pa.x, w0.w, g3);
+                g0 = mfma16(pa.y, w1.x, g0); g1 = mfma16(pa.y, w1.y, g1); g2 = mfma16(pa.y, w1.z, g2); g3 = mfma16(pa.y, w1.w, g3);
+                g0 = mfma16(pa.z, w2v.x, g0); g1 = mfma16(pa.z, w2v.y, g1); g2 = mfma16(pa.z, w2v.z, g2); g3 = mfma16(pa.z, w2v.w, g3);
+                g0 = mfma16(pa.w, w3.x, g0); g1 = mfma16(pa.w, w3.y, g1); g2 = mfma16(pa.w, w3.z, g2); g3 = mfma16(pa.w, w3.w, g3);
+            } else {
+                const Planes4 pap = split_quad<edge_planes(NP)>(pa.x, pa.y, pa.z, pa.w);
+                g0 = mfma16_planes<NP>(pap, wp0, g0); g1 = mfma16_planes<NP>(pap, wp1, g1);
+                g2 = mfma16_planes<NP>(pap, wp2, g2); g3 = mfma16_planes<NP>(pap, wp3, g3);
+            }
+            float* trow = tile + 4 * q * SEND_LD + 4 * r;
+            *reinterpret_cast<float4*>(trow) = send_row(wd4, cur_ops.dd0, cur_ops.a0, cur_ops.b0, g0[0], g1[0], g2[0], g3[0]);
+            *reinterpret_cast<float4*>(trow + SEND_LD) = send_row(wd4, cur_ops.dd1, cur_ops.a1, cur_ops.b1, g0[1], g1[1], g2[1], g3[1]);
+            *reinterpret_cast<float4*>(trow + 2 * SEND_LD) = send_row(wd4, cur_ops.dd2, cur_ops.a2, cur_ops.b2, g0[2], g1[2], g2[2], g3[2]);
+            *reinterpret_cast<float4*>(trow + 3 * SEND_LD) = send_row(wd4, cur_ops.dd3, cur_ops.a3, cur_ops.b3, g0[3], g1[3], g2[3], g3[3]);
         } else {
-            const Planes4 pap = split_quad<edge_planes(NP)>(pa.x, pa.y, pa.z, pa.w);
-            g0 = mfma16_planes<NP>(pap, wp0, g0); g1 = mfma16_planes<NP>(pap, wp1, g1);
-            g2 = mfma16_planes<NP>(pap, wp2, g2); g3 = mfma16_planes<NP>(pap, wp3, g3);
-        }
-        float* trow = tile + 4 * q * SEND_LD + 4 * r;
-        *reinterpret_cast<float4*>(trow) = send_row(wd4, cur_ops.dd0, cur_ops.a0, cur_ops.b0, g0[0], g1[0], g2[0], g3[0]);
-        *reinterpret_cast<float4*>(trow + SEND_LD) = send_row(wd4, cur_ops.dd1, cur_ops.a1, cur_ops.b1, g0[1], g1[1], g2[1], g3[1]);
-        *reinterpret_cast<float4*>(trow + 2 * SEND_LD) = send_row(wd4, cur_ops.dd2, cur_ops.a2, cur_ops.b2, g0[2], g1[2], g2[2], g3[2]);
-        *reinterpret_cast<float4*>(trow + 3 * SEND_LD) = send_row(wd4, cur_ops.dd3, cur_ops.a3, cur_ops.b3, g0[3], g1[3], g2[3], g3[3]);
+            if constexpr (NP == 6) {
+                g0 = mfma16(pa.x, w0, g0);
+                g0 = mfma16(pa.y, w1, g0);
+                g0 = mfma16(pa.z, w2v, g0);
+                g0 = mfma16(pa.w, w3, g0);
+            } else {
+                g0 = mfma16_planes<NP>(split_quad<edge_planes(NP)>(pa.x, pa.y, pa.z, pa.w), wp0, g0);
+            }
+            float* trow = tile + 4 * q * SEND_LD + r;
+            trow[0] = send_row(wd4, cur_ops.dd0, cur_ops.a0, cur_ops.b0, g0[0]);
+            trow[SEND_LD] = send_row(wd4, cur_ops.dd1, cur_ops.a1, cur_ops.b1, g0[1]);
+            trow[2 * SEND_LD] = send_row(wd4, cur_ops.dd2, cur_ops.a2, cur_ops.b2, g0[2]);
+            trow[3 * SEND_LD] = send_row(wd4, cur_ops.dd3, cur_ops.a3, cur_ops.b3, g0[3]);
+        }
         float v[KNB];
 #pragma unroll
-        for (int row = 0; row < KNB; ++row) v[row] = tile[row * SEND_LD + lane];
+        for (int row = 0; row < KNB; ++row) v[row] = owner ? tile[row * SEND_LD + lane] : 0.f;
         const int rows = (p_end - p0 < KNB) ? (p_end - p0) : KNB;
 #pragma unroll
         for (int row = 0; row < KNB; ++row) {
             if (row < rows) {
                 while (p0 + row >= cur_end) {
-                    drow[(int64_t)cur * 2 * Hp] = run;
+                    if (owner) drow[(int64_t)cur * 2 * Hp] = run;
                     run = 0.f;
                     ++cur;
                     if (cur - rp_base >= 64) {
@@ -760,9 +959,32 @@
         __builtin_amdgcn_sched_barrier(0);
     }
     for (; cur < s_end; ++cur) {
-        drow[(int64_t)cur * 2 * Hp] = run;
+        if (owner) drow[(int64_t)cur * 2 * Hp] = run;
         run = 0.f;
     }
+}
+
+template <int NP>
+__global__ void __launch_bounds__(THREADS)
+k_edge_bwd_send(const float* __restrict__ ab, const float* __restrict__ wd, const float* __restrict__ w2,
+                const float* __restrict__ dpre2, const int* __restrict__ t_rowptr, const int4* __restrict__ rec,
+                float* __restrict__ dab, int N, int Hp, BwTiles bt, int chunks, int n_items, int remap) {
+    __shared__ __attribute__((aligned(16))) float s_tile[WAVES][KNB * SEND_LD];
+    const int lane = threadIdx.x & 63;
+    const int wave = __builtin_amdgcn_readfirstlane(threadIdx.x >> 6);
+    const int item = xcd_item((int)blockIdx.x, (int)gridDim.x, n_items, remap);
+    if (item < 0) return;
+    int s_beg, s_end;
+    if (item >= bt.full * chunks) {
+        const int first = bt.full * chunks;
+        send_share(t_rowptr, N, (item - first) * WAVES + wave, (n_items - first) * WAVES, lane, s_beg, s_end);
+        if (bt.narrow) send_range<NP, 1>(s_tile[wave], ab, wd, w2, dpre2, t_rowptr, rec, dab, N, Hp, bt.full, s_beg, s_end, lane);
+        if (bt.z0 >= 0)
+            for (int sj = s_beg; sj < s_end; ++sj) zero_columns(dab + (int64_t)sj * 2 * Hp + Hp, 0, 1, bt.z0, Hp, lane);
+        return;
+    }
+    send_share(t_rowptr, N, (item / bt.full) * WAVES + wave, chunks * WAVES, lane, s_beg, s_end);
+    send_range<NP, 4>(s_tile[wave], ab, wd, w2, dpre2, t_rowptr, rec, dab, N, Hp, item % bt.full, s_beg, s_end, lane);
 }
 
 inline int edge_xcd_remap() {
@@ -866,23 +1088,25 @@
 }
 
 static inline int prep_blocks(int64_t N) { return eqh_grid_for(N, WAVES, 2048); }
+static inline int bw_ws_chunks(int64_t N, int tiles) { return bw_chunks(N, tiles > 1 ? tiles - 1 : 1); }
 
 extern "C" size_t egnn_edge_bwd_workspace_bytes(int64_t N, int32_t Hp) {
     if (N < 0 || Hp <= 0) return 0;
-    const int chunks = bw_chunks(N, Hp >> 6);
+    const int chunks = bw_ws_chunks(N, Hp >> 6);
     return ((size_t)chunks * (size_t)(MDIM + 1) * (size_t)Hp + (size_t)(N > 0 ? N : 1) * 256 +
             (size_t)(N > 0 ? N : 1) * KNB * 4 + (size_t)prep_blocks(N) * MDIM) * sizeof(float);
 }
 
-extern "C" int egnn_edge_bwd_p(const float* ab, const float* wd, const float* w2, const int32_t* nbr,
+extern "C" int egnn_edge_bwd_h(const float* ab, const float* wd, const float* w2, const int32_t* nbr,
                                const float* d2, const float* pre2, const float* dm, int64_t dm_ld,
                                const int32_t* t_rowptr, const int32_t* t_perm, int64_t N, int32_t Hp,
                                float* dab, float* dwd, float* dw2, float* dpre2, float* db2,
-                               int32_t db2_accumulate, int32_t dw_accumulate, void* workspace, size_t workspace_bytes,
-                               void* stream_, int32_t products) {
+                               int32_t db2_accumulate, int32_t dw_accumulate, int32_t h_live, void* workspace,
+                               size_t workspace_bytes, void* stream_, int32_t products) {
     if (products != 6 && products != 3 && products != 1) return EQH_ERR_ARG;
     int rc = check_common(N, Hp);
     if (rc) return rc;
+    if (h_live <= 0 || h_live > Hp) return EQH_ERR_ARG;
     if (!dwd || !dw2) return EQH_ERR_ARG;
     hipStream_t stream = static_cast<hipStream_t>(stream_);
     if (N == 0) {
@@ -900,13 +1124,18 @@
         return EQH_ERR_ALIGN;
     if (workspace_bytes < egnn_edge_bwd_workspace_bytes(N, Hp)) return EQH_ERR_ARG;
     if (dm_ld < MDIM || (dm_ld & 3)) return EQH_ERR_ARG;
-    const int tiles = Hp >> 6;
-    const int chunks = bw_chunks(N, tiles);
+    BwTiles bt = bw_tiles(Hp, h_live), bt_s = bt;
+    const int ws_chunks = bw_ws_chunks(N, Hp >> 6);
+    int chunks = bw_chunks_live(N, bt, RECV_SPAN_MAX);
+    if (chunks > ws_chunks) chunks = ws_chunks;
     const int chunk_items = (int)((N + chunks - 1) / chunks);
     const int used = (int)((N + chunk_items - 1) / chunk_items);
+    const int n_items = used * bt.full + bw_tail_items(bt, used);
+    const int chunks_s = bw_chunks_live(N, bt_s, SEND_SPAN_MAX);
+    const int n_items_s = chunks_s * bt_s.full + bw_tail_items(bt_s, chunks_s);
     float* slab_w2 = static_cast<float*>(workspace);
     float* slab_wd = slab_w2 + (size_t)MDIM * Hp;
-    float* dpre2_t = slab_w2 + (size_t)chunks * (MDIM + 1) * Hp;
+    float* dpre2_t = slab_w2 + (size_t)ws_chunks * (MDIM + 1) * Hp;
     int4* rec = reinterpret_cast<int4*>(dpre2_t + (size_t)N * 256);
     float* slab_b2 = db2 ? reinterpret_cast<float*>(rec + (size_t)N * KNB) : nullptr;
     const int pblocks = prep_blocks(N);
@@ -920,14 +1149,24 @@
     const int remap = edge_xcd_remap();
     const auto recv = products == 6 ? k_edge_bwd_recv<6> : (products == 3 ? k_edge_bwd_recv<3> : k_edge_bwd_recv<1>);
     const auto send = products == 6 ? k_edge_bwd_send<6> : (products == 3 ? k_edge_bwd_send<3> : k_edge_bwd_send<1>);
-    hipLaunchKernelGGL(recv, dim3(xcd_grid(used * tiles, remap)), dim3(THREADS), 0, stream, ab, wd, w2, nbr, d2, dpre2,
-                       dpre2_t, dab, slab_w2, slab_wd, (int)N, (int)Hp, tiles, chunk_items, used * tiles, remap);
+    hipLaunchKernelGGL(recv, dim3(xcd_grid(n_items, remap)), dim3(THREADS), 0, stream, ab, wd, w2, nbr, d2, dpre2,
+                       dpre2_t, dab, slab_w2, slab_wd, (int)N, (int)Hp, bt, used, chunk_items, n_items, remap);
     EQH_CHECK_LAUNCH();
-    hipLaunchKernelGGL(send, dim3(xcd_grid(used * tiles, remap)), dim3(THREADS), 0, stream, ab, wd, w2, dpre2, t_rowptr,
-                       rec, dab, (int)N, (int)Hp, tiles, chunk_items, used * tiles, remap);
+    hipLaunchKernelGGL(send, dim3(xcd_grid(n_items_s, remap)), dim3(THREADS), 0, stream, ab, wd, w2, dpre2, t_rowptr,
+                       rec, dab, (int)N, (int)Hp, bt_s, chunks_s, n_items_s, remap);
     EQH_CHECK_LAUNCH();
     return eqh_reduce_slabs3_async(slab_w2, used, (int64_t)(MDIM + 1) * Hp, dw2, dwd, dwd, (int64_t)MDIM * Hp, Hp,
                                    dw_accumulate ? 1 : 0, stream);
+}
+
+extern "C" int egnn_edge_bwd_p(const float* ab, const float* wd, const float* w2, const int32_t* nbr,
+                               const float* d2, const float* pre2, const float* dm, int64_t dm_ld,
+                               const int32_t* t_rowptr, const int32_t* t_perm, int64_t N, int32_t Hp,
+                               float* dab, float* dwd, float* dw2, float* dpre2, float* db2,
+                               int32_t db2_accumulate, int32_t dw_accumulate, void* workspace, size_t workspace_bytes,
+                               void* stream_, int32_t products) {
+    return egnn_edge_bwd_h(ab, wd, w2, nbr, d2, pre2, dm, dm_ld, t_rowptr, t_perm, N, Hp, dab, dwd, dw2, dpre2, db2,
+                           db2_accumulate, dw_accumulate, Hp, workspace, workspace_bytes, stream_, products);
 }
 
 extern "C" int egnn_edge_bwd(const float* ab, const float* wd, const float* w2, const int32_t* nbr,
diff --git a/equihgnn_amd/layers.py b/equihgnn_amd/layers.py
--- a/equihgnn_amd/layers.py
+++ b/equihgnn_amd/layers.py
@@ -393,7 +393,7 @@
             ab, normed, res = ops.egnn_feats(feats, w_cat, b_cat, nn_)
         else:
             ab, normed, res = ops.linear(feats, w_cat, b_cat), nn_(feats), feats
-        m_i = ops.egnn_edge(ab, w_d, w2, lin2.bias, nbr, d2, csr_t)
+        m_i = ops.egnn_edge(ab, w_d, w2, lin2.bias, nbr, d2, csr_t, hdim)
         ops.signal_point()
         if fold:
             return ops.egnn_node_mlp_ln(normed, m_i, n0, n3, nn_)
diff --git a/equihgnn_amd/ops/egnn.py b/equihgnn_amd/ops/egnn.py
--- a/equihgnn_amd/ops/egnn.py
+++ b/equihgnn_amd/ops/egnn.py
@@ -17,12 +17,15 @@
 class _EgnnEdge(torch.autograd.Function):
 
     @staticmethod
-    def forward(ctx, ab, wd, w2, b2, nbr, d2, csr_t: CSR, b2_param=None, w_refs=None):
+    def forward(ctx, ab, wd, w2, b2, nbr, d2, csr_t: CSR, b2_param=None, w_refs=None, h_live=None):
         _require_gpu(ab, "egnn_edge")
         ab, wd, w2, b2 = _f32c(ab), _f32c(wd), _f32c(w2), _f32c(b2)
         N, Hp = ab.shape[0], ab.shape[1] // 2
         if nbr.shape != (N, 16) or w2.shape != (16, Hp) or wd.shape != (Hp,) or b2.shape != (16,):
             raise ValueError("egnn_edge: shapes must be ab[N,2Hp] wd[Hp] w2[16,Hp] b2[16] nbr[N,16]")
+        if h_live is not None and not 0 < h_live <= Hp:
+            raise ValueError(f"egnn_edge: h_live = {h_live} outside (0, {Hp}]")
+        ctx.h_live = None if h_live is None or h_live == Hp else int(h_live)
         m = torch.empty((N, 16), dtype=torch.float32, device=ab.device)
         pre2 = torch.empty((N, 16, 16), dtype=torch.float32, device=ab.device)
         ctx.products = products = precision.edge_products()
@@ -50,14 +53,15 @@
         ws = _workspace(ws_bytes, dev)
         tg = _acc_target(ctx.b2_param)
         db2 = tg if tg is not None else torch.empty(16, dtype=torch.float32, device=dev)
+        head = (_ptr(ab), _ptr(wd), _ptr(w2), _ptr(ctx.nbr), _ptr(ctx.d2), _ptr(pre2), _ptr(dm), dm_ld, _ptr(ctx.csr_t.rowptr),
+                _ptr(ctx.csr_t.perm), N, Hp, _ptr(dab), _ptr(dwd), _ptr(dw2), _ptr(dpre2), _ptr(db2), 1 if tg is not None else 0,
+                1 if w_acc else 0)
+        tail = (_ptr(ws), ws_bytes, _stream(dev), ctx.products)
         timed("egnn_edge_bwd", N * 16 * Hp * 96,
-              lambda: hip.check(L.egnn_edge_bwd_p(_ptr(ab), _ptr(wd), _ptr(w2), _ptr(ctx.nbr), _ptr(ctx.d2), _ptr(pre2),
-                                                  _ptr(dm), dm_ld, _ptr(ctx.csr_t.rowptr), _ptr(ctx.csr_t.perm), N, Hp, _ptr(dab),
-                                                  _ptr(dwd), _ptr(dw2), _ptr(dpre2), _ptr(db2), 1 if tg is not None else 0,
-                                                  1 if w_acc else 0, _ptr(ws), ws_bytes, _stream(dev), ctx.products),
-                                "egnn_edge_bwd"))
+              lambda: hip.check(L.egnn_edge_bwd_p(*head, *tail) if ctx.h_live is None
+                                else L.egnn_edge_bwd_h(*head, ctx.h_live, *tail), "egnn_edge_bwd"))
         return (dab, None if w_acc else dwd, None if w_acc else dw2, (None if tg is not None else db2), None, None, None, None,
-                None)
+                None, None)
 
 
 class _EgnnFeats(torch.autograd.Function):
@@ -214,9 +218,9 @@
     return tuple(leaves)
 
 
-def egnn_edge(ab, wd, w2, b2, nbr, d2, csr_t: CSR):
+def egnn_edge(ab, wd, w2, b2, nbr, d2, csr_t: CSR, h_live=None):
     _note_acc(b2)
-    return _EgnnEdge.apply(ab, wd, w2, b2, nbr, d2, csr_t, b2, (wd, w2))
+    return _EgnnEdge.apply(ab, wd, w2, b2, nbr, d2, csr_t, b2, (wd, w2), h_live)
 
 
 NODE_WGRAD_BLOCKS = not os.environ.get("EQH_NO_NODE_WGRAD_BLOCKS")
diff --git a/include/equihgnn_hip.h b/include/equihgnn_hip.h
--- a/include/equihgnn_hip.h
+++ b/include/equihgnn_hip.h
@@ -335,6 +335,11 @@
                     const int32_t* t_perm, int64_t N, int32_t Hp, float* dab, float* dwd, float* dw2,
                     float* dpre2, float* db2, int32_t db2_accumulate, int32_t dw_accumulate, void* workspace,
                     size_t workspace_bytes, void* stream, int32_t products);
+int egnn_edge_bwd_h(const float* ab, const float* wd, const float* w2, const int32_t* nbr,
+                    const float* d2, const float* pre2, const float* dm, int64_t dm_ld, const int32_t* t_rowptr,
+                    const int32_t* t_perm, int64_t N, int32_t Hp, float* dab, float* dwd, float* dw2,
+                    float* dpre2, float* db2, int32_t db2_accumulate, int32_t dw_accumulate, int32_t h_live,
+                    void* workspace, size_t workspace_bytes, void* stream, int32_t products);
 
 int hg_rowgemm_fwd(const float* z, const float* w, const int32_t* rowptr, const int32_t* perm,
                    int64_t R, int32_t Kd, int32_t L, float* out, int32_t accumulate, void* stream);
```

New measurement: 229,100 molecules/s, median of 6. About the same (+0.2%).
